# Gardlin/PCR-CG

Measured on AMD Instinct MI355X. Metric: fragment-pairs/s KPFCNN+GCN fwd, 30k-pt pairs, higher is better.
Workload: dtype f32

## Files before the change

include/pcrcg.h:

```cpp
#ifndef PCRCG_H
#define PCRCG_H

#include <stddef.h>
#include <stdint.h>

#ifdef __cplusplus
extern "C" {
#endif

#define PCRCG_OK 0
#define PCRCG_EBADARG (-1)
#define PCRCG_EWORKSPACE (-2)
#define PCRCG_ELAUNCH (-3)
#define PCRCG_ECAPACITY (-4)

#define PCRCG_KPOINTS 15

const char* pcrcg_last_error(void);
#define PCRCG_ABI_VERSION 4
int pcrcg_abi_version(void);

int pcrcg_debug_set(const char* spec);
int pcrcg_debug_release(void);

// ... 1 lines not shown
int pcrcg_grid_subsample_batch(const float* pts, int n, const int* len, int nb, float dl, int max_p,
                               float* out_pts, int* out_len, int* out_m, void* ws, size_t ws_bytes,
                               void* stream);

size_t pcrcg_umap_order_ws_bytes(int m);
int pcrcg_umap_order(const uint64_t* keys, int m, int* order, void* ws, size_t ws_bytes, void* stream);

size_t pcrcg_cellgrid_ws_bytes(int ns, int nb);
int pcrcg_cellgrid_build(const float* sup, int ns, const int* slen, int nb, float radius, void* grid,
                         size_t grid_bytes, void* stream);
int pcrcg_radius_query(const float* q, int nq, const int* qlen, int ns, const int* slen, int nb,
                       float radius, const void* grid, int cols, int64_t* out_idx, int* out_count,
                       int* out_max_count, int* status, void* stream);
int pcrcg_radius_query_ex(const float* q, int nq, const int* qlen, int ns, const int* slen, int nb,
                          float radius, const void* grid, int cols, int64_t* out_idx, int* out_count,
                          int* out_max_count, int* status, int* out_tie_rows, int* out_tie_count, void* stream);
int pcrcg_radius_query_groups(const float* q, int nq, const int* qlen, int ns, const int* slen, int nb, int group,
                              float radius, const void* grid, int cols, int64_t* out_idx, int* out_count,
                              int* out_max_count, int* status, int* out_tie_rows, int* out_tie_count, void* stream);
int pcrcg_radius_query_cells(const void* qgrid, const float* q, int nq, const int* qlen, const void* sgrid, int ns,
                             const int* slen, int nb, int group, float radius, int cols, int64_t* out_idx, int* out_count,
                             int* out_max_count, int* status, int* out_tie_rows, int* out_tie_count, void* stream);
size_t pcrcg_radius_neighbors_ws_bytes(int ns, int nb);
int pcrcg_radius_neighbors_batch(const float* q, int nq, const float* sup, int ns, const int* qlen,
                                 const int* slen, int nb, float radius, int cols, int64_t* out_idx,
                                 int* out_count, int* out_max_count, int* status, void* ws,
                                 size_t ws_bytes, void* stream);

#define PCRCG_MAX_REORDER_JOBS 12
typedef struct pcrcg_reorder_job {
    const float* q;
    const int* qlen;
    const int* rows;
    const int* count;
    int64_t* idx;
    int nq, nbq, cloud0, nrows, max_count, cols;
    float radius;
    int group;
    const float* sup;
    const void* forest;
    int forest_ns, forest_nb;
} pcrcg_reorder_job;
size_t pcrcg_kdforest_ws_bytes(int ns, int nb);
int pcrcg_kdforest_build(const float* sup, int ns, const int* slen, int nb, void* forest, size_t forest_bytes,
                         void* stream);
int pcrcg_radius_reorder(const float* q, int nq, const int* qlen, int nbq, const float* sup, int ns, int nb,
                         const void* forest, int cloud0, float radius, const int* rows, int nrows, const int* count,
                         int max_count, int cols, int64_t* idx, int* status, void* stream);
int pcrcg_radius_reorder_jobs(const pcrcg_reorder_job* jobs, int njobs, const float* sup, int ns, int nb,
                              const void* forest, int* status, void* stream);

size_t pcrcg_kpconv_ws_bytes(int ns);
int pcrcg_kpconv_aggregate(const float* q_pts, int nq, const float* s_pts, int ns, const int64_t* idx,
                           int h, int ld_idx, const float* x, int cin, const float* kp, float extent,
                           float* wf, float* inv_n, void* ws, size_t ws_bytes, void* stream);
int pcrcg_kpconv_aggregate_bf16(const float* q_pts, int nq, const float* s_pts, int ns, const int64_t* idx, int h,
                                int ld_idx, const float* x, int cin, const float* kp, float extent, void* x_bf16,
                                void* wf_bf16, float* inv_n, void* ws, size_t ws_bytes, void* stream);

void pcrcg_profile_kpconv(int enable);
int pcrcg_profile_kpconv_read(float* ms, int* nq, int* h, int* cin, int* cout, int* kind, int cap);

int pcrcg_gemm_f32(const float* a, int lda, const float* b, int ldb, int trans_b, float* c, int ldc, int m,
                   int n, int k, const float* row_scale, const float* bias, void* stream);
size_t pcrcg_gemm_colstats_bytes(int m, int n);
int pcrcg_gemm_f32_colstats(const float* a, int lda, const float* b, int ldb, int trans_b, float* c, int ldc,
                            int m, int n, int k, const float* row_scale, const float* bias, void* colstats,
                            size_t colstats_bytes, int* h_chunks, void* stream);
int pcrcg_gemm_bf16a_f32_colstats(const void* a_bf16, int lda, const float* b, int ldb, float* c, int ldc, int m, int n,
                                  int k, const float* row_scale, const float* bias, void* colstats,
                                  size_t colstats_bytes, int* h_chunks, void* stream);

int pcrcg_gemm_f32_fused(const float* a, int lda, const int64_t* idx, int ld_idx, int ns, const float* zero_row,
                         const void* a_sums, double a_count, float a_eps, float a_slope, const float* b, int ldb,
                         const float* bias, float* c, int ldc, int m, int n, int k, int accumulate, void* stream);

void pcrcg_gemm_set_mode(int mode);
int pcrcg_gemm_get_mode(void);
int pcrcg_gemm_redo_counts(unsigned long long* out2, int reset);
void pcrcg_thread_shares_gpu(int on);

int pcrcg_gather_max(const float* x, int ns, int c, const int64_t* idx, int nq, int h, int ld_idx,
                     float* out, void* stream);
int pcrcg_gather_first(const float* x, int ns, int c, const int64_t* idx, int nq, int ld_idx, float* out,
                       int ld_out, void* stream);
size_t pcrcg_instnorm_ws_bytes(int c);
int pcrcg_instnorm_stats_from_partials(const void* partials, int chunks, int c, double count, float eps,
                                       float* stats, void* stream);
int pcrcg_instnorm_stats(const float* x, int n, int c, int ldx, float eps, float* stats, void* ws,
                         size_t ws_bytes, void* stream);
int pcrcg_instnorm_apply(const float* x, int n, int c, int ldx, const float* stats, const float* res,
                         int ldr, const float* res_stats, float slope, float* y, int ldy, void* stream);
int pcrcg_instnorm_colsums(const float* x, int n, int c, int ldx, void* sums, void* stream);
int pcrcg_instnorm_apply_sums(const float* x, int n, int c, int ldx, const void* sums, double count, float eps,
                              const float* res, int ldr, const void* res_sums, float slope, float* y, int ldy,
                              void* stream);

int pcrcg_fill2d(float* dst, int ld, int rows, int cols, float value, void* stream);
int pcrcg_inject_image_features(const float* fmap, int c, int h, int w, const float* valid, const int64_t* inds2d,
                                const int64_t* inds3d, int n, long row_offset, long n_rows, float* x, int ldx,
                                void* stream);

typedef struct pcrcg_image_frame {
    const float* fmap;
    const float* depth;
    const float* valid;
    float world2camera[16];
    float intrinsics[16];
    float thresh;
    int h, w;
    int depth_h, depth_w;
    int target;
} pcrcg_image_frame;

size_t pcrcg_project_depth_ws_bytes(int n);
int pcrcg_project_depth(const float* points, int n, const float* depth, int h, int w, const float* h_world2camera,
                        const float* h_intrinsics, float thresh, int64_t* inds2d, int64_t* inds3d, int* k, void* ws,
                        size_t ws_bytes, void* stream);
int pcrcg_inject_frames(const float* points, long n_points, long len_src, const pcrcg_image_frame* h_frames, int n_frames,
                        int c, float* x, int ldx, void* stream);
int pcrcg_superglue_valid_maps(const float* keypoints0, int n0, const float* keypoints1, int n1, const int64_t* matches,
                               const float* confidence, int window, int map_w, int map_h, float* src_valid, float* tgt_valid,
                               void* stream);

int pcrcg_knn(const float* coords, int n, int k, int* idx, void* stream);
size_t pcrcg_edgeconv_ws_bytes(int c);
int pcrcg_edgeconv_reduce(const float* ctr, int ld_ctr, const float* nbr, int ld_nbr, const int* idx,
                          int n, int k, int c, float eps, float* emax, int ld_emax, float* stats,
                          void* ws, size_t ws_bytes, void* stream);
int pcrcg_edgeconv_reduce_sums(const float* ctr, int ld_ctr, const float* nbr, int ld_nbr, const int* idx, int n, int k,
                               int c, float* emax, int ld_emax, void* sums, void* stream);
int pcrcg_softmax_rows(float* x, int rows, int cols, int ld, float scale, void* stream);
int pcrcg_attention_supported(int d);
int pcrcg_attention(const float* q, int ldq, const float* k, int ldk, const float* v, int ldv, float* out, int ldo, int n,
                    int ms, int heads, int d, float scale, void* stream);
int pcrcg_softmax_matvec(const float* x, int rows, int cols, int ld, float scale, const float* vec, int ldv, float* y,
                         int ldy, void* stream);

int pcrcg_check_status(const int* status, void* stream);

int pcrcg_copy2d(const float* src, int ld_src, float* dst, int ld_dst, int rows, int cols, void* stream);
int pcrcg_add(const float* a, const float* b, float* dst, long n, void* stream);
int pcrcg_l2norm_rows(const float* src, int ld_src, float* dst, int ld_dst, int rows, int cols, void* stream);
int pcrcg_sigmoid_scores(const float* src, int ld_src, float* dst, int rows, void* stream);

#define PCRCG_MAX_LEVELS 8
#define PCRCG_MAX_BLOCKS 32
#define PCRCG_MAX_GNN 8

enum { PCRCG_BLK_SIMPLE = 0, PCRCG_BLK_RESNETB = 1, PCRCG_BLK_UNARY = 2, PCRCG_BLK_LAST_UNARY = 3,
       PCRCG_BLK_UPSAMPLE = 4 };

typedef struct pcrcg_block {
    int type;
    int layer;
    int strided;
    int in_dim, out_dim;
    int mid_dim;
    float extent;
    const float* kp;
    const float* kp_w;
    const float* kp_wt;
    const float* kp_w_pad;
    int cin_pad;
    const float* unary1;
    const float* unary2;
    const float* shortcut;
    const float* mlp;
    int mlp_ld;
    const float* mlp_skip;
    int mlp_skip_ld, skip_dim;
} pcrcg_block;

typedef struct pcrcg_gnn_layer {
    int cross;
    const float* edge1;
    const float* edge2;
    const float* conv3;
    const float *wq, *bq, *wk, *bk, *wv, *bv;
    const float *wm, *bm;
    const float *w0, *b0;
    const float *w3, *b3;
} pcrcg_gnn_layer;

typedef struct pcrcg_model {
    int n_enc, n_dec, n_gnn;
    pcrcg_block enc[PCRCG_MAX_BLOCKS];
    pcrcg_block dec[PCRCG_MAX_BLOCKS];
    pcrcg_gnn_layer gnn[PCRCG_MAX_GNN];
    int enc_skip[PCRCG_MAX_BLOCKS];
    int dec_concat[PCRCG_MAX_BLOCKS];
    int enc_out_dim, gnn_dim, heads, knn_k, final_dim;
    const float *bottle_w, *bottle_b;
    const float *proj_gnn_w, *proj_gnn_b;
    const float *proj_score_w, *proj_score_b;
    float temperature;
    int feature_bf16;
} pcrcg_model;

typedef struct pcrcg_table { const int64_t* idx; int rows, cols, ld; } pcrcg_table;

typedef struct pcrcg_batch {
    int n_levels;
    const float* points[PCRCG_MAX_LEVELS];
    int n_points[PCRCG_MAX_LEVELS];
    pcrcg_table neighbors[PCRCG_MAX_LEVELS], pools[PCRCG_MAX_LEVELS], upsamples[PCRCG_MAX_LEVELS];
    const float* features;
    int feat_dim;
    int len_src_c;
    const int* stack_lengths[PCRCG_MAX_LEVELS];
} pcrcg_batch;

typedef struct pcrcg_outputs {
    float* feats_f;
    float* scores_overlap;
    float* scores_saliency;
} pcrcg_outputs;

size_t pcrcg_kpfcnn_ws_bytes(const pcrcg_model* model, const pcrcg_batch* batch);
int pcrcg_kpfcnn_forward(const pcrcg_model* model, const pcrcg_batch* batch, const pcrcg_outputs* out, void* ws,
                         size_t ws_bytes, void* stream);

size_t pcrcg_kpfcnn_group_ws_bytes(const pcrcg_model* model, const pcrcg_batch* batches, int n);
int pcrcg_kpfcnn_forward_group(const pcrcg_model* model, const pcrcg_batch* batches, const pcrcg_outputs* outs, int n,
                               void* ws, size_t ws_bytes, void* stream);

typedef struct pcrcg_pyramid_cfg {
    int n_levels;
    float r_conv[PCRCG_MAX_LEVELS], r_pool[PCRCG_MAX_LEVELS], dl[PCRCG_MAX_LEVELS];
    int has_conv[PCRCG_MAX_LEVELS], pooled[PCRCG_MAX_LEVELS], limit[PCRCG_MAX_LEVELS];
    int tie_order;
    int group;
    int up_nearest;
    double shrink;
    void* side_stream;
    void* side_stream2;
} pcrcg_pyramid_cfg;
typedef struct pcrcg_pyramid_restore {
    int njobs;
    pcrcg_reorder_job jobs[PCRCG_MAX_REORDER_JOBS];
    int* tie_status;
} pcrcg_pyramid_restore;
size_t pcrcg_pyramid_ws_bytes(int n0, int nb, const pcrcg_pyramid_cfg* cfg);
int pcrcg_pyramid_build(const float* pts, int n0, const int* len, int nb, const pcrcg_pyramid_cfg* cfg, void* ws,
                        size_t ws_bytes, int* h_scratch, pcrcg_batch* out, int* h_lengths, int* h_status,
                        pcrcg_pyramid_restore* deferred, void* stream);
int pcrcg_pyramid_build_parts(const float* const* pts_parts, const int* n_parts, const int* const* len_parts,
                              const int* nb_parts, int parts, const pcrcg_pyramid_cfg* cfg, void* ws, size_t ws_bytes,
                              int* h_scratch, pcrcg_batch* out, int* h_lengths, int* h_status,
                              pcrcg_pyramid_restore* deferred, void* stream);
int pcrcg_pyramid_restore_run(const pcrcg_pyramid_restore* r, int* h_status, void* stream);

int pcrcg_stream_create(void** stream, int priority);
int pcrcg_stream_destroy(void* stream);
int pcrcg_stream_pipe_classes(void* const* streams, int n, int* cls, void* scratch);

typedef struct pcrcg_ransac_trace {
    int* samples;
    int* pass;
    float* xf32;
    double* xf64;
    int* valid_ids;
    int* counts;
    double* sums;
} pcrcg_ransac_trace;

size_t pcrcg_ransac_ws_bytes(int n, int m, int max_iteration, int max_validation);
int pcrcg_feature_match(const float* src_feat, int ld_src, int n, const float* tgt_feat, int ld_tgt, int m, int c, int mutual,
                        int* corr, int* k, void* ws, size_t ws_bytes, void* stream);
int pcrcg_ransac(const float* src, int n, const float* tgt, int m, const void* grid, const int* corr, int k_max, const int* k,
                 int ransac_n, double threshold, double edge_similarity, int distance_check, int max_iteration,
                 int max_validation, uint64_t seed, double* out_transform, double* out_stats, const pcrcg_ransac_trace* trace,
                 void* ws, size_t ws_bytes, void* stream);

size_t pcrcg_ransac_batch_ws_bytes(int B, int n_total, int m_total, int max_iteration, int max_validation);
int pcrcg_feature_match_batch(const float* src_feat, int ld_src, const int* src_off, int n_total, int n_max,
                              const float* tgt_feat, int ld_tgt, const int* tgt_off, int m_total, int m_max, int c, int B,
                              int* corr, int* k, void* ws, size_t ws_bytes, void* stream);
int pcrcg_ransac_batch(const float* src, const int* src_off, const float* tgt, const int* tgt_off, int m_total, const void* grid,
                       const int* corr, const int* k, int B, int ransac_n, double threshold, double edge_similarity,
                       int distance_check, int max_iteration, int max_validation, const uint64_t* seeds,
                       double* out_transform, double* out_stats, void* ws, size_t ws_bytes, void* stream);

size_t pcrcg_inlier_stats_batch_ws_bytes(int B, int n_total, int m_total);
int pcrcg_inlier_stats_batch(const float* src, const float* src_feat, int ld_src, const int* src_off, int n_total, int n_max,
                             const float* tgt, const float* tgt_feat, int ld_tgt, const int* tgt_off, int m_total, int m_max,
                             int c, int B, const float* rt, const float* thr, int n_thr, int* counts, int* k_mutual,
                             float* dist, int* mutual, int* arg_s, int* arg_t, void* ws, size_t ws_bytes, void* stream);


size_t pcrcg_chamfer_batch_ws_bytes(int B, int n_total, int m_total, int r_total);
int pcrcg_chamfer_batch(const float* src, const int* src_off, int n_total, const float* ref, const int* ref_off, int m_total,
                        const float* raw, const int* raw_off, int r_total, int B, const float* pred, const float* gt,
// ... 15 lines not shown
```

pcrcg_amd/_lib.py:

```python
import ctypes
import os

_HERE = os.path.dirname(os.path.abspath(__file__))
LIB_PATH = os.path.join(_HERE, "libpcrcg_hip.so")


def lib_identity():
    import hashlib
    with open(LIB_PATH, "rb") as f:
        return LIB_PATH, hashlib.sha256(f.read()).hexdigest()[:16]

ABI_VERSION = 4

c_int, c_float, c_void_p, c_size_t = ctypes.c_int, ctypes.c_float, ctypes.c_void_p, ctypes.c_size_t

SIGNATURES = {
    "pcrcg_last_error": (ctypes.c_char_p, []),
    "pcrcg_abi_version": (c_int, []),
    "pcrcg_debug_set": (c_int, [ctypes.c_char_p]),
    "pcrcg_check_status": (c_int, [c_void_p, c_void_p]),
    "pcrcg_grid_subsample_ws_bytes": (c_size_t, [c_int, c_int]),
    "pcrcg_grid_subsample_batch": (c_int, [c_void_p, c_int, c_void_p, c_int, c_float, c_int, c_void_p, c_void_p,
                                           c_void_p, c_void_p, c_size_t, c_void_p]),
    "pcrcg_umap_order_ws_bytes": (c_size_t, [c_int]),
    "pcrcg_umap_order": (c_int, [c_void_p, c_int, c_void_p, c_void_p, c_size_t, c_void_p]),
    "pcrcg_cellgrid_ws_bytes": (c_size_t, [c_int, c_int]),
    "pcrcg_cellgrid_build": (c_int, [c_void_p, c_int, c_void_p, c_int, c_float, c_void_p, c_size_t, c_void_p]),
    "pcrcg_radius_query": (c_int, [c_void_p, c_int, c_void_p, c_int, c_void_p, c_int, c_float, c_void_p, c_int,
                                   c_void_p, c_void_p, c_void_p, c_void_p, c_void_p]),
    "pcrcg_radius_query_ex": (c_int, [c_void_p, c_int, c_void_p, c_int, c_void_p, c_int, c_float, c_void_p, c_int,
                                      c_void_p, c_void_p, c_void_p, c_void_p, c_void_p, c_void_p, c_void_p]),
    "pcrcg_radius_query_groups": (c_int, [c_void_p, c_int, c_void_p, c_int, c_void_p, c_int, c_int, c_float, c_void_p, c_int,
                                          c_void_p, c_void_p, c_void_p, c_void_p, c_void_p, c_void_p, c_void_p]),
    "pcrcg_radius_query_cells": (c_int, [c_void_p, c_void_p, c_int, c_void_p, c_void_p, c_int, c_void_p, c_int, c_int, c_float,
                                         c_int, c_void_p, c_void_p, c_void_p, c_void_p, c_void_p, c_void_p, c_void_p]),
    "pcrcg_kdforest_ws_bytes": (c_size_t, [c_int, c_int]),
    "pcrcg_kdforest_build": (c_int, [c_void_p, c_int, c_void_p, c_int, c_void_p, c_size_t, c_void_p]),
    "pcrcg_radius_reorder": (c_int, [c_void_p, c_int, c_void_p, c_int, c_void_p, c_int, c_int, c_void_p, c_int,
                                     c_float, c_void_p, c_int, c_void_p, c_int, c_int, c_void_p, c_void_p, c_void_p]),
    "pcrcg_radius_reorder_jobs": (c_int, [c_void_p, c_int, c_void_p, c_int, c_int, c_void_p, c_void_p, c_void_p]),
    "pcrcg_radius_neighbors_ws_bytes": (c_size_t, [c_int, c_int]),
    "pcrcg_radius_neighbors_batch": (c_int, [c_void_p, c_int, c_void_p, c_int, c_void_p, c_void_p, c_int, c_float,
                                             c_int, c_void_p, c_void_p, c_void_p, c_void_p, c_void_p, c_size_t,
                                             c_void_p]),
    "pcrcg_kpconv_ws_bytes": (c_size_t, [c_int]),
    "pcrcg_kpconv_aggregate": (c_int, [c_void_p, c_int, c_void_p, c_int, c_void_p, c_int, c_int, c_void_p, c_int,
                                       c_void_p, c_float, c_void_p, c_void_p, c_void_p, c_size_t, c_void_p]),
    "pcrcg_kpconv_aggregate_bf16": (c_int, [c_void_p, c_int, c_void_p, c_int, c_void_p, c_int, c_int, c_void_p, c_int,
                                            c_void_p, c_float, c_void_p, c_void_p, c_void_p, c_void_p, c_size_t,
                                            c_void_p]),
    "pcrcg_profile_kpconv": (None, [c_int]),
    "pcrcg_profile_kpconv_read": (c_int, [c_void_p, c_void_p, c_void_p, c_void_p, c_void_p, c_void_p, c_int]),
    "pcrcg_gemm_f32": (c_int, [c_void_p, c_int, c_void_p, c_int, c_int, c_void_p, c_int, c_int, c_int, c_int,
                               c_void_p, c_void_p, c_void_p]),
    "pcrcg_gemm_colstats_bytes": (c_size_t, [c_int, c_int]),
    "pcrcg_gemm_f32_colstats": (c_int, [c_void_p, c_int, c_void_p, c_int, c_int, c_void_p, c_int, c_int, c_int, c_int,
                                        c_void_p, c_void_p, c_void_p, c_size_t, c_void_p, c_void_p]),
    "pcrcg_gemm_bf16a_f32_colstats": (c_int, [c_void_p, c_int, c_void_p, c_int, c_void_p, c_int, c_int, c_int, c_int,
                                              c_void_p, c_void_p, c_void_p, c_size_t, c_void_p, c_void_p]),
    "pcrcg_gemm_f32_fused": (c_int, [c_void_p, c_int, c_void_p, c_int, c_int, c_void_p, c_void_p, ctypes.c_double, c_float,
                                     c_float, c_void_p, c_int, c_void_p, c_void_p, c_int, c_int, c_int, c_int, c_int, c_void_p]),
    "pcrcg_gemm_set_mode": (None, [c_int]),
    "pcrcg_gemm_get_mode": (c_int, []),
    "pcrcg_gemm_redo_counts": (c_int, [c_void_p, c_int]),
    "pcrcg_instnorm_stats_from_partials": (c_int, [c_void_p, c_int, c_int, ctypes.c_double, c_float, c_void_p,
                                                   c_void_p]),
    "pcrcg_gather_max": (c_int, [c_void_p, c_int, c_int, c_void_p, c_int, c_int, c_int, c_void_p, c_void_p]),
    "pcrcg_gather_first": (c_int, [c_void_p, c_int, c_int, c_void_p, c_int, c_int, c_void_p, c_int, c_void_p]),
    "pcrcg_instnorm_ws_bytes": (c_size_t, [c_int]),
    "pcrcg_instnorm_stats": (c_int, [c_void_p, c_int, c_int, c_int, c_float, c_void_p, c_void_p, c_size_t, c_void_p]),
    "pcrcg_instnorm_apply": (c_int, [c_void_p, c_int, c_int, c_int, c_void_p, c_void_p, c_int, c_void_p, c_float,
                                     c_void_p, c_int, c_void_p]),
    "pcrcg_instnorm_colsums": (c_int, [c_void_p, c_int, c_int, c_int, c_void_p, c_void_p]),
    "pcrcg_instnorm_apply_sums": (c_int, [c_void_p, c_int, c_int, c_int, c_void_p, ctypes.c_double, c_float, c_void_p, c_int,
                                          c_void_p, c_float, c_void_p, c_int, c_void_p]),
    "pcrcg_fill2d": (c_int, [c_void_p, c_int, c_int, c_int, c_float, c_void_p]),
    "pcrcg_inject_image_features": (c_int, [c_void_p, c_int, c_int, c_int, c_void_p, c_void_p, c_void_p, c_int, ctypes.c_long,
                                            ctypes.c_long, c_void_p, c_int, c_void_p]),
    "pcrcg_project_depth_ws_bytes": (c_size_t, [c_int]),
    "pcrcg_project_depth": (c_int, [c_void_p, c_int, c_void_p, c_int, c_int, c_void_p, c_void_p, c_float, c_void_p, c_void_p,
                                    c_void_p, c_void_p, c_size_t, c_void_p]),
    "pcrcg_inject_frames": (c_int, [c_void_p, ctypes.c_long, ctypes.c_long, c_void_p, c_int, c_int, c_void_p, c_int, c_void_p]),
    "pcrcg_superglue_valid_maps": (c_int, [c_void_p, c_int, c_void_p, c_int, c_void_p, c_void_p, c_int, c_int, c_int, c_void_p,
                                           c_void_p, c_void_p]),
    "pcrcg_knn": (c_int, [c_void_p, c_int, c_int, c_void_p, c_void_p]),
    "pcrcg_edgeconv_ws_bytes": (c_size_t, [c_int]),
    "pcrcg_edgeconv_reduce": (c_int, [c_void_p, c_int, c_void_p, c_int, c_void_p, c_int, c_int, c_int, c_float,
                                      c_void_p, c_int, c_void_p, c_void_p, c_size_t, c_void_p]),
    "pcrcg_edgeconv_reduce_sums": (c_int, [c_void_p, c_int, c_void_p, c_int, c_void_p, c_int, c_int, c_int, c_void_p, c_int,
                                           c_void_p, c_void_p]),
    "pcrcg_softmax_rows": (c_int, [c_void_p, c_int, c_int, c_int, c_float, c_void_p]),
    "pcrcg_attention_supported": (c_int, [c_int]),
    "pcrcg_attention": (c_int, [c_void_p, c_int, c_void_p, c_int, c_void_p, c_int, c_void_p, c_int, c_int, c_int, c_int,
                                c_int, c_float, c_void_p]),
    "pcrcg_softmax_matvec": (c_int, [c_void_p, c_int, c_int, c_int, c_float, c_void_p, c_int, c_void_p, c_int, c_void_p]),
    "pcrcg_copy2d": (c_int, [c_void_p, c_int, c_void_p, c_int, c_int, c_int, c_void_p]),
    "pcrcg_add": (c_int, [c_void_p, c_void_p, c_void_p, ctypes.c_long, c_void_p]),
    "pcrcg_l2norm_rows": (c_int, [c_void_p, c_int, c_void_p, c_int, c_int, c_int, c_void_p]),
    "pcrcg_sigmoid_scores": (c_int, [c_void_p, c_int, c_void_p, c_int, c_void_p]),
    "pcrcg_kpfcnn_ws_bytes": (c_size_t, [c_void_p, c_void_p]),
    "pcrcg_kpfcnn_group_ws_bytes": (c_size_t, [c_void_p, c_void_p, c_int]),
    "pcrcg_kpfcnn_forward_group": (c_int, [c_void_p, c_void_p, c_void_p, c_int, c_void_p, c_size_t, c_void_p]),
    "pcrcg_kpfcnn_forward": (c_int, [c_void_p, c_void_p, c_void_p, c_void_p, c_size_t, c_void_p]),
    "pcrcg_pyramid_ws_bytes": (c_size_t, [c_int, c_int, c_void_p]),
    "pcrcg_pyramid_build": (c_int, [c_void_p, c_int, c_void_p, c_int, c_void_p, c_void_p, c_size_t, c_void_p, c_void_p,
                                    c_void_p, c_void_p, c_void_p, c_void_p]),
    "pcrcg_pyramid_build_parts": (c_int, [c_void_p, c_void_p, c_void_p, c_void_p, c_int, c_void_p, c_void_p, c_size_t, c_void_p,
                                          c_void_p, c_void_p, c_void_p, c_void_p, c_void_p]),
    "pcrcg_pyramid_restore_run": (c_int, [c_void_p, c_void_p, c_void_p]),
    "pcrcg_debug_release": (c_int, []),
    "pcrcg_stream_pipe_classes": (c_int, [c_void_p, c_int, c_void_p, c_void_p]),
    "pcrcg_thread_shares_gpu": (None, [c_int]),
    "pcrcg_stream_create": (c_int, [c_void_p, c_int]),
    "pcrcg_stream_destroy": (c_int, [c_void_p]),
    "pcrcg_ransac_ws_bytes": (c_size_t, [c_int, c_int, c_int, c_int]),
    "pcrcg_feature_match": (c_int, [c_void_p, c_int, c_int, c_void_p, c_int, c_int, c_int, c_int, c_void_p, c_void_p,
                                    c_void_p, c_size_t, c_void_p]),
    "pcrcg_ransac": (c_int, [c_void_p, c_int, c_void_p, c_int, c_void_p, c_void_p, c_int, c_void_p, c_int, ctypes.c_double,
                             ctypes.c_double, c_int, c_int, c_int, ctypes.c_uint64, c_void_p, c_void_p, c_void_p, c_void_p,
                             c_size_t, c_void_p]),
    "pcrcg_ransac_batch_ws_bytes": (c_size_t, [c_int, c_int, c_int, c_int, c_int]),
    "pcrcg_feature_match_batch": (c_int, [c_void_p, c_int, c_void_p, c_int, c_int, c_void_p, c_int, c_void_p, c_int, c_int,
                                          c_int, c_int, c_void_p, c_void_p, c_void_p, c_size_t, c_void_p]),
    "pcrcg_ransac_batch": (c_int, [c_void_p, c_void_p, c_void_p, c_void_p, c_int, c_void_p, c_void_p, c_void_p, c_int, c_int,
                                   ctypes.c_double, ctypes.c_double, c_int, c_int, c_int, c_void_p, c_void_p, c_void_p,
                                   c_void_p, c_size_t, c_void_p]),
    "pcrcg_inlier_stats_batch_ws_bytes": (c_size_t, [c_int, c_int, c_int]),
    "pcrcg_inlier_stats_batch": (c_int, [c_void_p, c_void_p, c_int, c_void_p, c_int, c_int, c_void_p, c_void_p, c_int, c_void_p,
                                         c_int, c_int, c_int, c_int, c_void_p, c_void_p, c_int, c_void_p, c_void_p, c_void_p,
                                         c_void_p, c_void_p, c_void_p, c_void_p, c_size_t, c_void_p]),
    "pcrcg_chamfer_batch_ws_bytes": (c_size_t, [c_int, c_int, c_int, c_int]),
    "pcrcg_chamfer_batch": (c_int, [c_void_p, c_void_p, c_int, c_void_p, c_void_p, c_int, c_void_p, c_void_p, c_int, c_int,
                                    c_void_p, c_void_p, c_void_p, c_void_p, c_void_p, c_void_p, c_void_p, c_void_p, c_void_p,
                                    c_void_p, c_size_t, c_void_p]),
    "pcrcg_res50unet_arena_bytes": (c_size_t, [c_int]),
    "pcrcg_res50unet_pack": (c_int, [c_void_p, c_int, c_int, c_void_p, c_void_p]),
    "pcrcg_res50unet_ws_bytes": (c_size_t, [c_int, c_int, c_int]),
    "pcrcg_res50unet_forward": (c_int, [c_void_p, c_void_p, c_int, c_int, c_void_p, c_int, c_int, c_int, c_int, c_int,
                                        c_void_p, c_void_p, c_size_t, c_void_p]),
    "pcrcg_gemm_f32_ex": (c_int, [c_void_p, c_int, c_int, c_void_p, c_int, c_int, c_void_p, c_int, c_int, c_int, c_int,
                                  c_void_p, c_void_p, c_void_p]),
    "pcrcg_gemm_f32_grad": (c_int, [c_void_p, c_int, c_int, c_void_p, c_int, c_int, c_void_p, c_int, c_int, c_int, c_int,
                                  c_void_p, c_void_p, c_int, c_void_p]),
    "pcrcg_kpconv_backward_dx": (c_int, [c_void_p, c_int, c_void_p, c_int, c_void_p, c_int, c_int, c_void_p, c_int,
                                         c_void_p, c_float, c_void_p, c_void_p]),
    "pcrcg_kpconv_forward_ws_bytes": (c_size_t, [c_int, c_int, c_int]),
    "pcrcg_kpconv_forward": (c_int, [c_void_p, c_int, c_void_p, c_int, c_void_p, c_int, c_int, c_void_p, c_int, c_void_p,
                                     c_float, c_void_p, c_int, c_void_p, c_int, c_void_p, c_size_t, c_void_p]),
    "pcrcg_kpconv_backward_ws_bytes": (c_size_t, [c_int, c_int, c_int]),
    "pcrcg_kpconv_backward": (c_int, [c_void_p, c_int, c_void_p, c_int, c_void_p, c_int, c_int, c_int, c_void_p, c_float,
# ... 68 lines not shown
```

pcrcg_amd/csrc/common.h:

```cpp
#pragma once
#include <hip/hip_runtime.h>

#include <cstdarg>
#include <cstdint>
#include <cstdio>
#include <mutex>

#include "pcrcg.h"

namespace pcrcg {

void set_error(const char* fmt, ...);

inline hipStream_t as_stream(void* s) { return reinterpret_cast<hipStream_t>(s); }

struct Carver {
    char* base;
    size_t cap;
    size_t off = 0;
    Carver(void* ws, size_t bytes) : base(static_cast<char*>(ws)), cap(bytes) {}
    template <typename T>
    T* take(size_t count) {
        size_t bytes = (count * sizeof(T) + 255) & ~size_t(255);
        T* p = reinterpret_cast<T*>(base + off);
// ... 5 lines not shown
inline size_t carve_bytes(size_t count, size_t elem) { return (count * elem + 255) & ~size_t(255); }

size_t scan_ws_bytes(int n);
int exclusive_scan_i32(const int* in, int* out, int n, int* total, void* ws, hipStream_t stream);

constexpr int kWave = 64;

int grid_subsample_bound(const float* pts, int n_bound, const int* len, int nb, float dl, int max_p, float* out_pts,
                         int* out_len, int* out_m, int out_cap, int* overflow, void* ws, size_t ws_bytes, hipStream_t stream);

bool instnorm_pack_ok(int c, int ldx, int ldy);
int instnorm_apply_pack(const float* x, int n, int c, int ldx, const float* stats, const double* sums, double count, float eps,
                        float slope, float* y, int ldy, const float* s_pts, float4* pk, hipStream_t st);
float4* kpconv_pk_ptr(void* ws, size_t ws_bytes, int ns);

void gemm_x6_release_det();
void trainops_release_det();
void conv2d_release_det();

int kdforest_build_levels(const float* sup, int ns, const int* slen, int nb, int per_level, const int* level_base, void* forest,
                          size_t forest_bytes, hipStream_t stream);

int radius_fast_cap();
int radius_query_pass(const float* q, int nq, const int* qlen, int ns, const int* slen, int nb, int group, float radius,
                      const void* grid, int cols, int64_t* out_idx, int* out_count, int* out_max_count, int* status,
                      int* out_tie_rows, int* out_tie_count, hipStream_t st, int pass);

bool gemm_x6_shared();
void gemm_x6_set_shared(int on);
int radius_cells_pass(const void* qgrid, const float* q, int nq, const int* qlen, const void* sgrid, int ns, const int* slen,
                      int nb, int group, float radius, int cols, int64_t* out_idx, int* out_count, int* out_max_count,
                      int* status, int* out_tie_rows, int* out_tie_count, hipStream_t st, int pass);
constexpr int kRadiusRedoStatus = 4;

struct GemmExtra {
    const long long* a_idx = nullptr;
    int a_idx_ld = 0, a_ns = 0;
    const float* a_zero = nullptr;
    bool accumulate = false;
    const double* a_sums = nullptr;
    double a_count = 0.0;
    float a_eps = 1e-5f, a_slope = 1.0f;
    int grad_operand = 0;
};

struct GemmPair {
    const float* a = nullptr;
    float* c = nullptr;
    int m = 0;
    const float* row_scale = nullptr;
    void* colstats = nullptr;
    int* h_chunks = nullptr;
    bool c_zeroed = false;
    const long long* a_idx = nullptr;
    int a_ns = 0;
    const double* a_sums = nullptr;
    double a_count = 0.0;
};
struct GemmGroup {
    int n = 0;
    GemmPair p[3];
};

int kpconv_pack(const float* x, int ns, int cin, const float* s_pts, void* ws, size_t ws_bytes, hipStream_t st,
                unsigned short* x_bf16 = nullptr);
int kpconv_aggregate_rows(const float* q_pts, int nq, const float* s_pts, int ns, const int64_t* idx, int h, int ld_idx,
                          const float* x, int cin, const float* kp, float extent, float* wf, float* inv_n, void* ws,
                          size_t ws_bytes, hipStream_t st, bool pack, bool stream_out, int c1_ld = 0);
int kpconv_aggregate_bf16(const float* q_pts, int nq, const float* s_pts, int ns, const int64_t* idx, int h, int ld_idx,
                          const float* x, unsigned short* x_bf16, int cin, const float* kp, float extent,
                          unsigned short* wf_bf16, float* inv_n, void* ws, size_t ws_bytes, hipStream_t st);

struct NormJob {
    const float* x; const double* sums; const float* res; const double* res_sums; float* y;
    const float* s_pts; float4* pk;
    int n; double count;
    float* stats_out = nullptr;
};
int instnorm_apply_sums_multi(const NormJob* jobs, int count, int c, int ldx, float eps, int ldr, float slope, int ldy, bool pack,
                              hipStream_t st);

struct GatherJob { const float* x; const int64_t* idx; float* out; int ns, nq, h, ld_idx; };
int gather_max_multi(const GatherJob* jobs, int count, int c, hipStream_t st);
int heads_multi(const float* const* x, const int* rows, int count, int ld, int fd, float* const* feats, float* const* s_ov,
                float* const* s_sal, hipStream_t st);
int copy2d_multi(const float* const* src, float* const* dst, const int* rows, int count, int ld_src, int ld_dst, int cols,
                 hipStream_t st);
int instnorm_colsums_multi(const float* const* x, double* const* sums, const int* n, int count, int c, int ldx, hipStream_t st);

struct EdgeCloud {
    const float* ctr; const float* nbr; const int* idx; float* emax; double* sums; int n, k;
};
bool edgeconv_rows_ok(const EdgeCloud* cl, int count, int ld_ctr, int ld_nbr, int ld_emax, int c);
int edgeconv_rows_multi(const EdgeCloud* cl, int count, int ld_ctr, int ld_nbr, int ld_emax, int c, bool atomic, int* nchunks_out,
                        hipStream_t st);

struct AttnCloud { const float* q; const float* k; const float* v; float* out; int n, ms; };
bool attention_mfma_ok(const AttnCloud* cl, int count, int ldq, int ldk, int ldv, int d);
int attention_mfma_multi(const AttnCloud* cl, int count, int ldq, int ldk, int ldv, int ldo, int heads, int d, float scale,
                         hipStream_t st);
bool attention_bwd_mfma_ok(int n, int ms, int d, int ldq, int ldk, int ldv, int ld_do);
int attention_bwd_mfma(const float* q, int ldq, const float* k, int ldk, const float* v, int ldv, const float* o, int ldo,
                       const float* d_o, int ld_do, float* dq, int ld_dq, float* dk, int ld_dk, float* dv, int ld_dv, int n, int ms,
                       int heads, int d, float scale, hipStream_t st);

struct DebugOpts {
    int stat_sums = 1;
    int stat_sums_rows = 1 << 30;
    int att_mfma = 1;
    int radius_blocks = 0;
    int kd_blocks = 0;
    int att_tq = 16;
    int kd_spin_limit = 0;
    int gemm_log = 0;
    int x6_tile = -1, x6_splitk = 0, x6_t1 = 1, x6_t2 = 1, x6_order = -1, x6_big = 0, x6_h2 = 1;
    int train_side_stream = 1;
    int gemm_tile = -1, gemm_splitk = 0, gemm_split_target = 768;
    int deterministic = 0;
    int bwd_mfma = 1;
};
const DebugOpts& debug_opts();

struct KpProfScope {
    hipStream_t st;
    hipEvent_t a, b;
    int nq, h, cin, cout, kind;
    bool on;
    KpProfScope(hipStream_t s, int nq, int h, int cin, int cout, int kind);
    ~KpProfScope();
};

}

#define PCRCG_CHECK_ARG(cond)                                                        \
    do {                                                                             \
        if (!(cond)) {                                                               \
            pcrcg::set_error("%s: bad argument: %s", __func__, #cond);               \
            return PCRCG_EBADARG;                                                    \
        }                                                                            \
    } while (0)

#define PCRCG_CHECK_WS(carver)                                                                     \
    do {                                                                                           \
        if (!(carver).ok()) {                                                                      \
            pcrcg::set_error("%s: workspace too small (%zu needed, %zu given)", __func__,          \
                             (carver).off, (carver).cap);                                          \
            return PCRCG_EWORKSPACE;                                                               \
        }                                                                                          \
    } while (0)

#define PCRCG_CHECK_HIP(expr)                                                                  \
    do {                                                                                       \
        hipError_t e_ = (expr);                                                                \
        if (e_ != hipSuccess) {                                                                \
            pcrcg::set_error("%s: %s failed: %s", __func__, #expr, hipGetErrorString(e_));     \
            return PCRCG_ELAUNCH;                                                              \
        }                                                                                      \
    } while (0)

#define PCRCG_CHECK_LAUNCH() PCRCG_CHECK_HIP(hipGetLastError())

namespace pcrcg {
inline hipError_t grant_max_dyn_lds(const void* kern) {
    hipFuncAttributes at;
    hipError_t e = hipFuncGetAttributes(&at, kern);
    if (e != hipSuccess) return e;
// ... 18 lines not shown
```

pcrcg_amd/csrc/pointops.hip:

```cpp
#include "common.h"

namespace pcrcg {
namespace {

constexpr int kWavesPerBlock = 4;

struct GatherMulti { const float* x[4]; const long long* idx[4]; float* out[4]; int ns[4], nq[4], h[4], ld_idx[4]; };
template <bool VEC4>
__global__ void __launch_bounds__(kWavesPerBlock * 64) k_gather_max(GatherMulti mm, int c, int nchunk) {
    const int g = blockIdx.y;
    const float* __restrict__ x = mm.x[g];
    const long long* __restrict__ idx = mm.idx[g];
    float* __restrict__ out = mm.out[g];
    const int ns = mm.ns[g], nq = mm.nq[g], h = mm.h[g], ld_idx = mm.ld_idx[g];
    const int lane = threadIdx.x & 63;
    const long item = (long)blockIdx.x * kWavesPerBlock + __builtin_amdgcn_readfirstlane((int)(threadIdx.x >> 6));
    if (item >= (long)nq * nchunk) return;
    const int q = (int)(item / nchunk), chunk = (int)(item - (long)q * nchunk);
    const long long* row = idx + (long)q * ld_idx;
    if (VEC4) {
        const int cb = chunk * 64 + lane;
        if (cb >= (c >> 2)) return;
        float4 m = make_float4(0.f, 0.f, 0.f, 0.f);
        bool any = false;
#pragma unroll 4
        for (int j = 0; j < h; ++j) {
            const long long i = row[j];
            float4 v = make_float4(0.f, 0.f, 0.f, 0.f);
            if (i >= 0 && i < ns) v = reinterpret_cast<const float4*>(x + i * c)[cb];
            if (!any) { m = v; any = true; }
            else { m.x = fmaxf(m.x, v.x); m.y = fmaxf(m.y, v.y); m.z = fmaxf(m.z, v.z); m.w = fmaxf(m.w, v.w); }
        }
        reinterpret_cast<float4*>(out + (long)q * c)[cb] = m;
    } else {
        const int cc = chunk * 64 + lane;
        if (cc >= c) return;
        float m = 0.f;
        bool any = false;
#pragma unroll 4
        for (int j = 0; j < h; ++j) {
            const long long i = row[j];
            const float v = (i >= 0 && i < ns) ? x[i * c + cc] : 0.f;
            m = any ? fmaxf(m, v) : v;
            any = true;
        }
        out[(long)q * c + cc] = m;
    }
}

__global__ void __launch_bounds__(256) k_gather_first(const float* __restrict__ x, int ns, int c,
                                                       const long long* __restrict__ idx, int nq, int ld_idx,
                                                       float* __restrict__ out, int ld_out) {
    const int lane = threadIdx.x & 63;
    const int q = blockIdx.x * 4 + __builtin_amdgcn_readfirstlane((int)(threadIdx.x >> 6));
    if (q >= nq) return;
    const long long i = idx[(long)q * ld_idx];
    const bool real = i >= 0 && i < ns;
    for (int cc = lane; cc < c; cc += 64) out[(long)q * ld_out + cc] = real ? x[i * c + cc] : 0.f;
}

constexpr int kStatChunks = 128;

struct ColsMulti { const float* x[4]; double* partial[4]; int n[4]; };
template <bool ATOMIC>
__global__ void __launch_bounds__(256) k_colstats_partial(ColsMulti mm, int c, int ldx) {
    const float* __restrict__ x = mm.x[blockIdx.z];
    double* __restrict__ partial = mm.partial[blockIdx.z];
    const int n = mm.n[blockIdx.z];
    __shared__ double s_sum[4][64], s_sq[4][64];
    const int lane = threadIdx.x & 63, rl = threadIdx.x >> 6;
    const int ch = blockIdx.y * 64 + lane;
    const int chunk = blockIdx.x, nchunks = gridDim.x;
    const long rows_per = ((long)n + nchunks - 1) / nchunks;
    const long r0 = chunk * rows_per, r1 = min((long)n, r0 + rows_per);
    double s = 0.0, sq = 0.0;
    if (ch < c) {
        long r = r0 + rl;
        for (; r + 12 < r1; r += 16) {
            const float v0 = x[r * ldx + ch], v1 = x[(r + 4) * ldx + ch], v2 = x[(r + 8) * ldx + ch],
                        v3 = x[(r + 12) * ldx + ch];
            s += ((double)v0 + (double)v1) + ((double)v2 + (double)v3);
            sq += ((double)v0 * v0 + (double)v1 * v1) + ((double)v2 * v2 + (double)v3 * v3);
        }
        for (; r < r1; r += 4) {
            const double v = (double)x[r * ldx + ch];
            s += v;
            sq += v * v;
        }
    }
    s_sum[rl][lane] = s;
    s_sq[rl][lane] = sq;
    __syncthreads();
    if (rl == 0 && ch < c) {
        s = (s_sum[0][lane] + s_sum[1][lane]) + (s_sum[2][lane] + s_sum[3][lane]);
        sq = (s_sq[0][lane] + s_sq[1][lane]) + (s_sq[2][lane] + s_sq[3][lane]);
        if (ATOMIC) {
            if (r0 < r1) {
                unsafeAtomicAdd(&partial[ch], s);
                unsafeAtomicAdd(&partial[(long)c + ch], sq);
            }
        } else {
            partial[(long)ch * nchunks + chunk] = s;
            partial[((long)c + ch) * nchunks + chunk] = sq;
        }
    }
}

__global__ void __launch_bounds__(256) k_colstats_final(const double* __restrict__ partial, int nchunks, int c,
                                                         double count, float eps, float* __restrict__ stats) {
    const int lane = threadIdx.x & 63;
    const int ch = blockIdx.x * (blockDim.x >> 6) + (threadIdx.x >> 6);
    if (ch >= c) return;
    double s = 0.0, sq = 0.0;
    for (int k = lane; k < nchunks; k += 64) {
        s += partial[(long)ch * nchunks + k];
        sq += partial[((long)c + ch) * nchunks + k];
    }
#pragma unroll
    for (int d = 32; d >= 1; d >>= 1) {
        s += __shfl_xor(s, d, 64);
        sq += __shfl_xor(sq, d, 64);
    }
    if (lane != 0) return;
    const double mean = s / count;
    double var = sq / count - mean * mean;
    if (var < 0.0) var = 0.0;
    stats[2 * ch] = (float)mean;
    stats[2 * ch + 1] = (float)(1.0 / sqrt(var + (double)eps));
}
// ... 187 lines not shown
    const int c4 = c / 4;
    if (stats) {
        const long total = (long)n * c4;
        hipLaunchKernelGGL(k_instnorm_apply4_pack, dim3((unsigned)((total + 255) / 256)), dim3(256), 0, st, x, n, c4, ldx, stats,
                           slope, y, ldy, s_pts, pk);
    } else {
        NormJob one{x, sums, nullptr, nullptr, y, s_pts, pk, n, count};
        return instnorm_apply_sums_multi(&one, 1, c, ldx, eps, 0, slope, ldy, true, st);
    }
    PCRCG_CHECK_LAUNCH();
    return PCRCG_OK;
}

int instnorm_apply_sums_multi(const NormJob* jobs, int count, int c, int ldx, float eps, int ldr, float slope, int ldy, bool pack,
                              hipStream_t st) {
    PCRCG_CHECK_ARG(jobs && count >= 1 && count <= 4 && c >= 4 && c % 4 == 0);
    const int c4 = c / 4;
    NormMulti mm;
    int nmax = 0;
    for (int g = 0; g < 4; ++g) {
        const NormJob& j = jobs[g < count ? g : 0];
        mm.x[g] = j.x; mm.sums[g] = j.sums; mm.res[g] = j.res; mm.res_sums[g] = j.res_sums; mm.y[g] = j.y;
        mm.s_pts[g] = j.s_pts; mm.pk[g] = j.pk; mm.n[g] = g < count ? j.n : 0; mm.count[g] = j.count;
        mm.stats_out[g] = g < count ? j.stats_out : nullptr;
        if (g < count) {
            PCRCG_CHECK_ARG(j.n >= 0 && j.x && j.sums && j.y && j.count >= 1.0);
            PCRCG_CHECK_ARG((j.res != nullptr) == (jobs[0].res != nullptr) && (j.res_sums != nullptr) == (jobs[0].res_sums != nullptr));
            nmax = j.n > nmax ? j.n : nmax;
        }
    }
    if (nmax == 0) return PCRCG_OK;
    const int rp = 256 / (c4 < 256 ? c4 : 256);
    int rows_per_block = rp * 8;
    while (rows_per_block > rp && (long)(nmax + rows_per_block - 1) / rows_per_block * count < 256) rows_per_block -= rp;
    const dim3 grid((unsigned)((nmax + rows_per_block - 1) / rows_per_block), count);
    if (pack)
        hipLaunchKernelGGL(k_instnorm_apply4_sums_pack, grid, dim3(256), 0, st, mm, c4, ldx, eps, slope, ldy, rows_per_block);
    else if (!jobs[0].res)
        hipLaunchKernelGGL(k_instnorm_apply4_sums<0>, grid, dim3(256), 0, st, mm, c4, ldx, eps, ldr, slope, ldy, rows_per_block);
    else if (!jobs[0].res_sums)
        hipLaunchKernelGGL(k_instnorm_apply4_sums<1>, grid, dim3(256), 0, st, mm, c4, ldx, eps, ldr, slope, ldy, rows_per_block);
    else
        hipLaunchKernelGGL(k_instnorm_apply4_sums<2>, grid, dim3(256), 0, st, mm, c4, ldx, eps, ldr, slope, ldy, rows_per_block);
    PCRCG_CHECK_LAUNCH();
    return PCRCG_OK;
}

size_t colstats_ws_bytes(int c) { return carve_bytes((size_t)kStatChunks * 2 * (size_t)(c > 0 ? c : 1), sizeof(double)); }

int colstats_finalize(const double* partial, int nchunks, int c, double count, float eps, float* stats,
                      hipStream_t st) {
    hipLaunchKernelGGL(k_colstats_final, dim3((c + 3) / 4), dim3(256), 0, st, partial, nchunks, c, count, eps, stats);
    PCRCG_CHECK_LAUNCH();
    return PCRCG_OK;
}
int colstats_chunks() { return kStatChunks; }

int gather_max_multi(const GatherJob* jobs, int count, int c, hipStream_t st) {
    PCRCG_CHECK_ARG(jobs && count >= 1 && count <= 4 && c >= 1);
    GatherMulti mm;
    bool vec = c % 4 == 0;
    int nq_max = 0;
    for (int g = 0; g < 4; ++g) {
        const GatherJob& j = jobs[g < count ? g : 0];
        mm.x[g] = j.x; mm.idx[g] = reinterpret_cast<const long long*>(j.idx); mm.out[g] = j.out;
        mm.ns[g] = j.ns; mm.nq[g] = g < count ? j.nq : 0; mm.h[g] = j.h; mm.ld_idx[g] = j.ld_idx;
        if (g < count) {
            PCRCG_CHECK_ARG(j.ns >= 0 && j.nq >= 0 && j.h >= 1 && j.ld_idx >= j.h && (j.nq == 0 || (j.x && j.idx && j.out)));
            vec = vec && ((reinterpret_cast<uintptr_t>(j.x) | reinterpret_cast<uintptr_t>(j.out)) & 15) == 0;
            nq_max = j.nq > nq_max ? j.nq : nq_max;
        }
    }
    if (nq_max == 0) return PCRCG_OK;
    const int per_wave = vec ? 256 : 64;
    const int nchunk = (c + per_wave - 1) / per_wave;
    const long items = (long)nq_max * nchunk;
    const dim3 grid((unsigned)((items + kWavesPerBlock - 1) / kWavesPerBlock), count);
    if (vec) hipLaunchKernelGGL(k_gather_max<true>, grid, dim3(kWavesPerBlock * 64), 0, st, mm, c, nchunk);
    else hipLaunchKernelGGL(k_gather_max<false>, grid, dim3(kWavesPerBlock * 64), 0, st, mm, c, nchunk);
    PCRCG_CHECK_LAUNCH();
    return PCRCG_OK;
}

int instnorm_colsums_multi(const float* const* x, double* const* sums, const int* n, int count, int c, int ldx, hipStream_t st) {
    PCRCG_CHECK_ARG(count >= 1 && count <= 4 && c >= 1 && ldx >= c);
    ColsMulti mm;
    int nmax = 0;
    for (int g = 0; g < 4; ++g) {
        const int k = g < count ? g : 0;
        PCRCG_CHECK_ARG(n[k] >= 1 && x[k] && sums[k]);
        mm.x[g] = x[k]; mm.partial[g] = sums[k]; mm.n[g] = n[k];
        if (g < count) nmax = n[k] > nmax ? n[k] : nmax;
    }
    int chunks = (nmax + 63) / 64;
    if (chunks > kStatChunks) chunks = kStatChunks;
    if (debug_opts().deterministic) chunks = 1;
    hipLaunchKernelGGL(k_colstats_partial<true>, dim3(chunks, (c + 63) / 64, count), dim3(256), 0, st, mm, c, ldx);
    PCRCG_CHECK_LAUNCH();
    return PCRCG_OK;
}

}

using namespace pcrcg;

extern "C" {

int pcrcg_gather_max(const float* x, int ns, int c, const int64_t* idx, int nq, int h, int ld_idx,
                     float* out, void* stream) {
    PCRCG_CHECK_ARG(ns >= 0 && c >= 1 && nq >= 0 && h >= 1 && ld_idx >= h);
    if (nq == 0) return PCRCG_OK;
    PCRCG_CHECK_ARG(x && idx && out);
    const GatherJob one{x, idx, out, ns, nq, h, ld_idx};
    return gather_max_multi(&one, 1, c, as_stream(stream));
}

int pcrcg_gather_first(const float* x, int ns, int c, const int64_t* idx, int nq, int ld_idx, float* out,
                       int ld_out, void* stream) {
    PCRCG_CHECK_ARG(ns >= 0 && c >= 1 && nq >= 0 && ld_idx >= 1 && ld_out >= c);
    if (nq == 0) return PCRCG_OK;
    PCRCG_CHECK_ARG(x && idx && out);
    hipLaunchKernelGGL(k_gather_first, dim3((nq + 3) / 4), dim3(256), 0, as_stream(stream), x, ns, c,
                       reinterpret_cast<const long long*>(idx), nq, ld_idx, out, ld_out);
    PCRCG_CHECK_LAUNCH();
    return PCRCG_OK;
}

size_t pcrcg_instnorm_ws_bytes(int c) { return colstats_ws_bytes(c); }

int pcrcg_instnorm_stats_from_partials(const void* partials, int chunks, int c, double count, float eps,
                                       float* stats, void* stream) {
    PCRCG_CHECK_ARG(partials && stats && chunks >= 1 && c >= 1 && count >= 1.0);
    return colstats_finalize(static_cast<const double*>(partials), chunks, c, count, eps, stats, as_stream(stream));
}

int pcrcg_instnorm_stats(const float* x, int n, int c, int ldx, float eps, float* stats, void* ws,
                         size_t ws_bytes, void* stream) {
    PCRCG_CHECK_ARG(n >= 1 && c >= 1 && ldx >= c && x && stats && ws);
    Carver cv(ws, ws_bytes);
    double* partial = cv.take<double>((size_t)kStatChunks * 2 * c);
    PCRCG_CHECK_WS(cv);
    hipStream_t st = as_stream(stream);
    {
        ColsMulti mm;
        for (int g = 0; g < 4; ++g) { mm.x[g] = x; mm.partial[g] = partial; mm.n[g] = n; }
        hipLaunchKernelGGL(k_colstats_partial<false>, dim3(kStatChunks, (c + 63) / 64, 1), dim3(256), 0, st, mm, c, ldx);
    }
    return colstats_finalize(partial, kStatChunks, c, (double)n, eps, stats, st);
}

int pcrcg_instnorm_colsums(const float* x, int n, int c, int ldx, void* sums, void* stream) {
    PCRCG_CHECK_ARG(n >= 1 && c >= 1 && ldx >= c && x && sums);
    const float* xs[1] = {x};
    double* ss[1] = {static_cast<double*>(sums)};
    return instnorm_colsums_multi(xs, ss, &n, 1, c, ldx, as_stream(stream));
}

int pcrcg_instnorm_apply_sums(const float* x, int n, int c, int ldx, const void* sums, double count, float eps,
                              const float* res, int ldr, const void* res_sums, float slope, float* y, int ldy,
                              void* stream) {
    PCRCG_CHECK_ARG(n >= 0 && c >= 4 && c % 4 == 0 && ldx >= c && ldy >= c && count >= 1.0);
    if (n == 0) return PCRCG_OK;
    PCRCG_CHECK_ARG(x && sums && y && (!res || ldr >= c) && (!res_sums || res));
    const int c4 = c / 4;
    auto al16 = [](const void* p) { return (reinterpret_cast<uintptr_t>(p) & 15) == 0; };
    PCRCG_CHECK_ARG((c4 <= 256 ? 256 % c4 == 0 : c4 % 256 == 0) && ldx % 4 == 0 && ldy % 4 == 0 && al16(x) && al16(y) &&
                    (!res || (ldr % 4 == 0 && al16(res))));
    NormJob one{x, static_cast<const double*>(sums), res, static_cast<const double*>(res_sums), y, nullptr, nullptr, n, count};
    return instnorm_apply_sums_multi(&one, 1, c, ldx, eps, ldr, slope, ldy, false, as_stream(stream));
}

int pcrcg_instnorm_apply(const float* x, int n, int c, int ldx, const float* stats, const float* res,
                         int ldr, const float* res_stats, float slope, float* y, int ldy, void* stream) {
    PCRCG_CHECK_ARG(n >= 0 && c >= 1 && ldx >= c && ldy >= c);
    if (n == 0) return PCRCG_OK;
    PCRCG_CHECK_ARG(x && stats && y);
    PCRCG_CHECK_ARG(!res || ldr >= c);
    auto al16 = [](const void* p) { return (reinterpret_cast<uintptr_t>(p) & 15) == 0; };
    const bool vec = c % 4 == 0 && ldx % 4 == 0 && ldy % 4 == 0 && al16(x) && al16(y) && al16(stats) &&
                     (!res || (ldr % 4 == 0 && al16(res))) && (!res_stats || al16(res_stats));
    if (vec) {
        const long total = (long)n * (c / 4);
        hipLaunchKernelGGL(k_instnorm_apply4, dim3((unsigned)((total + 255) / 256)), dim3(256), 0, as_stream(stream), x,
                           n, c / 4, ldx, stats, res, ldr, res_stats, slope, y, ldy);
    } else {
        const long total = (long)n * c;
        hipLaunchKernelGGL(k_instnorm_apply, dim3((unsigned)((total + 255) / 256)), dim3(256), 0, as_stream(stream), x,
                           n, c, ldx, stats, res, ldr, res_stats, slope, y, ldy);
    }
    PCRCG_CHECK_LAUNCH();
    return PCRCG_OK;
}
}
```

pcrcg_amd/csrc/pyramid.hip:

```cpp
#include <time.h>

#include <cmath>
#include <cstdlib>
#include <vector>

#include "common.h"

namespace pcrcg {
namespace {

inline double now_us() {
    timespec ts;
    clock_gettime(CLOCK_MONOTONIC, &ts);
    return ts.tv_sec * 1e6 + ts.tv_nsec * 1e-3;
}

__global__ void k_probe_many(int* sink, int spin) {
    int x = threadIdx.x;
    for (int i = 0; i < spin; ++i) x = x * 1664525 + 1013904223;
    if (x == 0x7fffffff) sink[0] = x;
}
__global__ void k_probe_tiny(int* sink) {
    if (threadIdx.x == 1234567) sink[1] = 1;
}
// ... 128 lines not shown
    int* metas = A.take<int>(meta_ints);
    int* m_dev = metas + MS * max_tables;
    int* overflow = m_dev + L;
    int* tie_status = overflow + 1;
    if (!A.ok()) return PCRCG_EWORKSPACE;

    std::vector<TableRec> tables;
    tables.reserve(max_tables);
    if (!dry) {
        PCRCG_CHECK_HIP(hipMemsetAsync(metas, 0, sizeof(int) * meta_ints, st));
        size_t row = 0, cloud = 0;
        for (int i = 0; i < in.count; ++i) {
            if (in.n[i] > 0)
                PCRCG_CHECK_HIP(hipMemcpyAsync(level_pts[0] + 3 * row, in.pts[i], sizeof(float) * 3 * (size_t)in.n[i], hipMemcpyDeviceToDevice, st));
            PCRCG_CHECK_HIP(hipMemcpyAsync(lens_all + cloud, in.len[i], sizeof(int) * in.nb[i], hipMemcpyDeviceToDevice, st));
            row += (size_t)in.n[i];
            cloud += (size_t)in.nb[i];
        }
        PCRCG_CHECK_HIP(hipMemsetD32Async(reinterpret_cast<hipDeviceptr_t>(feats), 0x3f800000, (size_t)(n0 > 0 ? n0 : 1), st));
    }

    hipStream_t sub_st = cfg->side_stream ? as_stream(cfg->side_stream) : st;
    hipStream_t f_st = cfg->side_stream2 ? as_stream(cfg->side_stream2) : sub_st;
    EventBox events;
    auto order = [&](hipStream_t a, hipStream_t b) -> int {
        if (a == b || dry) return PCRCG_OK;
        hipEvent_t ev;
        PCRCG_PROPAGATE(events.make(&ev));
        PCRCG_CHECK_HIP(hipEventRecord(ev, a));
        PCRCG_CHECK_HIP(hipStreamWaitEvent(b, ev, 0));
        return PCRCG_OK;
    };
    const bool one_forest = !want_ties || f_st == st || L < 2;
    void* forest[2] = {nullptr, nullptr};
    size_t forest_b[2] = {0, 0};
    int forest_ns[2] = {0, 0}, forest_nb[2] = {0, 0};
    int level_base[PCRCG_MAX_LEVELS] = {};
    auto build_forest = [&](int which) -> int {
        if (!want_ties || (which == 1 && L < 2)) return PCRCG_OK;
        const int first = which == 1 ? 1 : 0, last = which == 0 ? 0 : L - 1, slot = which == 1 ? 1 : 0;
        for (int l = first; l <= last; ++l) level_base[l - first] = (int)((level_pts[l] - level_pts[first]) / 3);
        forest_ns[slot] = level_base[last - first] + cap[last];
        forest_nb[slot] = (last - first + 1) * nb;
        forest_b[slot] = pcrcg_kdforest_ws_bytes(forest_ns[slot], forest_nb[slot]);
        forest[slot] = A.raw(forest_b[slot]);
        if (!A.ok()) return PCRCG_EWORKSPACE;
        if (dry) return PCRCG_OK;
        PCRCG_PROPAGATE(order(which == 0 ? st : sub_st, f_st));
        return kdforest_build_levels(level_pts[first], forest_ns[slot], lens_all + (size_t)first * nb, forest_nb[slot],
                                     last > first ? nb : 0, level_base, forest[slot], forest_b[slot], f_st);
    };

    auto add_table = [&](int kind, int level, int q_level, const void* grid, const void* qgrid, float radius, const float* q,
                         const int* qlen, int nq, int ns, const int* slen, int limit, int sup_level) -> int {
        TableRec t;
        t.kind = kind; t.level = level; t.q_level = q_level;
        t.idx = A.take<int64_t>((size_t)nq * limit);
        t.counts = want_ties ? A.take<int>((size_t)nq) : nullptr;
        t.ties = want_ties ? A.take<int>((size_t)nq) : nullptr;
        t.meta = metas + MS * tables.size();
        t.q = q; t.qlen = qlen; t.nq = nq; t.limit = limit; t.sup_level = sup_level; t.radius = radius;
        t.grid = grid; t.ns = ns; t.slen = slen; t.qgrid = qgrid;
        if (!A.ok()) return PCRCG_EWORKSPACE;
        if (!dry)
            PCRCG_PROPAGATE(radius_cells_pass(t.qgrid, q, nq, qlen, grid, ns, slen, nb, group, radius, limit, t.idx, t.counts,
                                              t.meta, t.meta + P, t.ties, want_ties ? t.meta + P + 1 : nullptr, st, 1));
        tables.push_back(t);
        return PCRCG_OK;
    };
    auto build_grid = [&](const float* sup, int ns, const int* slen, float radius, void** grid) -> int {
        const size_t gb = pcrcg_cellgrid_ws_bytes(ns, nb);
        *grid = A.raw(gb);
        if (!A.ok()) return PCRCG_EWORKSPACE;
        if (!dry) PCRCG_PROPAGATE(pcrcg_cellgrid_build(sup, ns, slen, nb, radius, *grid, gb, st));
        return PCRCG_OK;
    };

    const size_t sub_wsb = L > 1 ? pcrcg_grid_subsample_ws_bytes(cap[0], nb) : 0;
    void* sub_ws = L > 1 ? A.raw(sub_wsb) : nullptr;
    if (!A.ok()) return PCRCG_EWORKSPACE;

    void* carried = nullptr;
    float carried_r = 0.f;
    PCRCG_PROPAGATE(order(st, sub_st));
    if (!one_forest) PCRCG_PROPAGATE(build_forest(0));
    else if (L == 1) PCRCG_PROPAGATE(build_forest(0));
    for (int l = 0; l < L; ++l) {
        const int limit = cfg->limit[l];
        const float r_conv = cfg->r_conv[l], r_pool = cfg->r_pool[l];
        float* pts = level_pts[l];
        int* lens = lens_all + (size_t)l * nb;
        const int n = cap[l];
        void* grid = nullptr;
        float grid_r = 0.f;
        const bool pooled = cfg->pooled[l] && l + 1 < L;
        if (!pooled && l + 1 < L) {
            set_error("pcrcg_pyramid_build: level %d of %d is not pooled", l, L);
            return PCRCG_EBADARG;
        }
        if (pooled && !dry)
            PCRCG_PROPAGATE(grid_subsample_bound(pts, n, lens, nb, cfg->dl[l], 0, level_pts[l + 1], lens + nb, m_dev + l, cap[l + 1],
                                                 overflow, sub_ws, sub_wsb, sub_st));
        if (pooled && l + 2 == L) PCRCG_PROPAGATE(build_forest(one_forest ? 2 : 1));
        if (cfg->has_conv[l]) {
            if (carried && carried_r == r_conv) { grid = carried; grid_r = carried_r; }
            else { PCRCG_PROPAGATE(build_grid(pts, n, lens, r_conv, &grid)); grid_r = r_conv; }
            PCRCG_PROPAGATE(add_table(0, l, l, grid, grid, r_conv, pts, lens, n, n, lens, limit, l));
        }
        carried = nullptr;
        if (pooled) {
            float* sub = level_pts[l + 1];
            int* sub_len = lens + nb;
            const int m = cap[l + 1];
            if (grid == nullptr || grid_r != r_pool) {
                PCRCG_PROPAGATE(build_grid(pts, n, lens, r_pool, &grid));
                grid_r = r_pool;
            }
            PCRCG_PROPAGATE(order(sub_st, st));
            void* up_grid = nullptr;
            PCRCG_PROPAGATE(build_grid(sub, m, sub_len, 2 * r_pool, &up_grid));
            PCRCG_PROPAGATE(add_table(1, l, l + 1, grid, up_grid, r_pool, sub, sub_len, m, n, lens, limit, l));
            PCRCG_PROPAGATE(add_table(2, l, l, up_grid, grid, 2 * r_pool, pts, lens, n, m, sub_len, cfg->up_nearest ? 1 : limit, l + 1));
            carried = up_grid;
            carried_r = 2 * r_pool;
        }
    }
    if (dry) return PCRCG_OK;
    hipEvent_t forests_done = nullptr;
    if (want_ties && f_st != st) {
        PCRCG_PROPAGATE(events.make(&forests_done));
        PCRCG_CHECK_HIP(hipEventRecord(forests_done, f_st));
    }

    const int nt = (int)tables.size();
    const int meta_words = MS * max_tables + L + 1;
    PCRCG_PROPAGATE(fetch(h_scratch, metas, meta_words, lens_all, L * nb, st, enqueue));
    if (forests_done) PCRCG_CHECK_HIP(hipStreamWaitEvent(st, forests_done, 0));
    const int* hm = h_scratch + 1;
    if (hm[MS * max_tables + L] != 0) {
        set_error("pcrcg_pyramid_build: a level keeps more rows than pcrcg_pyramid_cfg::shrink = %.3f allows -- call again with a "
                  "larger bound (1.0 always fits)", cfg->shrink);
        return PCRCG_EWORKSPACE;
    }
    for (int i = 0; i < L * nb; ++i) h_lengths[i] = hm[meta_words + i];
    int level_n[PCRCG_MAX_LEVELS];
    for (int l = 0; l < L; ++l) {
        level_n[l] = 0;
        for (int c = 0; c < nb; ++c) level_n[l] += h_lengths[(size_t)l * nb + c];
    }
    {
        int redone = 0;
        for (int i = 0; i < nt; ++i) {
            int widest = 0;
            for (int p = 0; p < P; ++p) widest = hm[MS * i + p] > widest ? hm[MS * i + p] : widest;
            const bool handed_over = (hm[MS * i + P] & kRadiusRedoStatus) != 0;
            if (widest <= radius_fast_cap() && !handed_over) continue;
            const TableRec& t = tables[i];
            PCRCG_PROPAGATE(radius_query_pass(t.q, t.nq, t.qlen, t.ns, t.slen, nb, group, t.radius, t.grid, t.limit, t.idx,
                                              t.counts, t.meta, t.meta + P, t.ties, want_ties ? t.meta + P + 1 : nullptr, st,
                                              2));
            ++redone;
        }
        if (redone) PCRCG_PROPAGATE(fetch(h_scratch, metas, meta_words, lens_all, L * nb, st));
    }
    auto group_rows = [&](int l, int p, int* row0, int* rows) {
        const int c0 = group > 0 ? p * group : 0, c1 = group > 0 ? c0 + group : nb;
        int a = 0, r = 0;
        for (int c = 0; c < c1; ++c) (c < c0 ? a : r) += h_lengths[(size_t)l * nb + c];
        *row0 = a;
        *rows = r;
    };
    for (int p = 0; p < P; ++p) {
        pcrcg_batch& o = out[p];
        o.n_levels = L;
        int row0, rows;
        group_rows(0, p, &row0, &rows);
        o.features = feats + row0;
        o.feat_dim = 1;
        o.len_src_c = h_lengths[(size_t)(L - 1) * nb + (group > 0 ? p * group : 0)];
        for (int l = 0; l < L; ++l) {
            group_rows(l, p, &row0, &rows);
            o.points[l] = level_pts[l] + 3 * (size_t)row0;
            o.n_points[l] = rows;
            o.stack_lengths[l] = lens_all + (size_t)l * nb + (group > 0 ? p * group : 0);
            o.neighbors[l] = pcrcg_table{nullptr, rows, 0, 1};
            o.pools[l] = pcrcg_table{nullptr, 0, 0, 1};
            o.upsamples[l] = pcrcg_table{nullptr, 0, 0, 1};
        }
    }
    pcrcg_pyramid_restore local;
    pcrcg_pyramid_restore& R = deferred ? *deferred : local;
    R.njobs = 0;
    for (int i = 0; i < nt; ++i) {
        TableRec& t = tables[i];
        const int status = hm[MS * i + P], tie_rows = hm[MS * i + P + 1];
        if (status != 0) {
            set_error("pcrcg_pyramid_build: radius search capacity exceeded (table %d)", i);
            return PCRCG_ECAPACITY;
        }
        int widest = 0;
        for (int p = 0; p < P; ++p) {
            const int max_count = hm[MS * i + p];
            widest = max_count > widest ? max_count : widest;
            const int cols = max_count < t.limit ? (max_count > 0 ? max_count : 0) : t.limit;
            int row0, rows;
            group_rows(t.q_level, p, &row0, &rows);
            pcrcg_table tab{t.idx + (size_t)row0 * t.limit, rows, cols, t.limit};
            if (t.kind == 0) out[p].neighbors[t.level] = tab;
            else if (t.kind == 1) out[p].pools[t.level] = tab;
            else out[p].upsamples[t.level] = tab;
        }
        if (want_ties && widest > 0 && tie_rows > 0 && R.njobs < PCRCG_MAX_REORDER_JOBS) {
            pcrcg_reorder_job& j = R.jobs[R.njobs++];
            const int fi = (one_forest || t.sup_level == 0) ? 0 : 1;
            j.q = t.q; j.qlen = t.qlen; j.rows = t.ties; j.count = t.counts; j.idx = t.idx;
            j.nq = level_n[t.q_level]; j.nbq = nb; j.cloud0 = one_forest ? t.sup_level * nb : (fi == 0 ? 0 : (t.sup_level - 1) * nb);
            j.nrows = tie_rows;
            j.max_count = widest < 8192 ? widest : 8192;
            j.cols = t.limit; j.radius = t.radius; j.group = group;
            j.sup = level_pts[fi]; j.forest = forest[fi]; j.forest_ns = forest_ns[fi]; j.forest_nb = forest_nb[fi];
        }
    }
    R.tie_status = tie_status;
    if (!deferred) return pcrcg_pyramid_restore_run(&R, h_status, st);
    return PCRCG_OK;
}

extern "C" {

size_t pcrcg_pyramid_ws_bytes(int n0, int nb, const pcrcg_pyramid_cfg* cfg) {
    if (!cfg || n0 < 0 || nb < 1 || cfg->n_levels < 1 || cfg->n_levels > PCRCG_MAX_LEVELS) return 0;
    Arena A(nullptr, 0, true);
    const Parts none{nullptr, nullptr, nullptr, nullptr, 0};
    if (pyramid_run(none, n0, nb, cfg, A, nullptr, nullptr, nullptr, nullptr, nullptr, nullptr) != PCRCG_OK) return 0;
    return A.peak + 4096;
}

int pcrcg_stream_create(void** stream, int priority) {
    PCRCG_CHECK_ARG(stream != nullptr);
    hipStream_t st = nullptr;
    PCRCG_CHECK_HIP(hipStreamCreateWithPriority(&st, hipStreamNonBlocking, priority));
    *stream = st;
    return PCRCG_OK;
}

int pcrcg_stream_pipe_classes(void* const* streams, int n, int* cls, void* scratch) {
    PCRCG_CHECK_ARG(streams && cls && scratch && n >= 1 && n <= 64);
    int* sink = static_cast<int*>(scratch);
    PCRCG_CHECK_HIP(hipDeviceSynchronize());
    for (int i = 0; i < n; ++i) hipLaunchKernelGGL(k_probe_tiny, dim3(1), dim3(64), 0, as_stream(streams[i]), sink);
    PCRCG_CHECK_HIP(hipDeviceSynchronize());
    const int blocks = 2000000;
    double t0 = now_us();
    hipLaunchKernelGGL(k_probe_many, dim3(blocks), dim3(64), 0, as_stream(streams[0]), sink, 64);
    PCRCG_CHECK_HIP(hipStreamSynchronize(as_stream(streams[0])));
    const double big_us = now_us() - t0;
    if (big_us < 400.0) {
        set_error("pcrcg_stream_pipe_classes: the dispatch-bound probe kernel took only %.0f us", big_us);
        return PCRCG_ELAUNCH;
    }
    int reps[8], nrep = 0;
    auto shares = [&](int a, int b, bool* out) -> int {
        int yes = 0, no = 0;
        for (int trial = 0; trial < 10 && yes < 2 && no < 2; ++trial) {
            const double launch = now_us();
            hipLaunchKernelGGL(k_probe_many, dim3(blocks), dim3(64), 0, as_stream(streams[a]), sink, 64);
            const double start = now_us();
            while (now_us() - start < 150.0) {}
            const double a0 = now_us();
            hipLaunchKernelGGL(k_probe_tiny, dim3(1), dim3(64), 0, as_stream(streams[b]), sink);
            const double a1 = now_us();
// ... 86 lines not shown
```

pcrcg_amd/csrc/radius.hip:

```cpp
#include <hip/hip_ext.h>

#include "block_scan.h"
#include <cstdlib>

#include "common.h"
#include "cellgrid.h"

namespace pcrcg {
namespace {

constexpr int kListCapFast = 256;
constexpr int kListCapFull = 1024;
constexpr long long kRedoMark = -2;
constexpr int kQueryWaves = 4;
constexpr int kTieCap = 256;

constexpr int kRedoStatus = 4;
constexpr int kCellCand = 1024;
constexpr int kCellListCap = 128;
constexpr unsigned kPadKey = 0x7FFFFFFFu;
constexpr int kCellTieCap = 512;
constexpr int kCellMaxCells = 256;
constexpr int kCellQ = 64;

// ... 790 lines not shown
                          int* out_max_count, int* status, int* out_tie_rows, int* out_tie_count, void* stream) {
    return pcrcg_radius_query_groups(q, nq, qlen, ns, slen, nb, 0, radius, grid, cols, out_idx, out_count, out_max_count,
                                     status, out_tie_rows, out_tie_count, stream);
}

int pcrcg_radius_query_groups(const float* q, int nq, const int* qlen, int ns, const int* slen, int nb, int group,
                              float radius, const void* grid, int cols, int64_t* out_idx, int* out_count,
                              int* out_max_count, int* status, int* out_tie_rows, int* out_tie_count, void* stream) {
    return pcrcg::radius_query_pass(q, nq, qlen, ns, slen, nb, group, radius, grid, cols, out_idx, out_count, out_max_count,
                                    status, out_tie_rows, out_tie_count, as_stream(stream), 0);
}
}

namespace pcrcg {
int radius_fast_cap() { return kListCapFast; }

int radius_query_pass(const float* q, int nq, const int* qlen, int ns, const int* slen, int nb, int group, float radius,
                      const void* grid, int cols, int64_t* out_idx, int* out_count, int* out_max_count, int* status,
                      int* out_tie_rows, int* out_tie_count, hipStream_t st, int pass) {
    PCRCG_CHECK_ARG(nq >= 0 && ns >= 0 && nb >= 1 && cols >= 1 && group >= 0);
    PCRCG_CHECK_ARG((out_tie_rows == nullptr) == (out_tie_count == nullptr));
    PCRCG_CHECK_ARG(qlen && slen && grid && out_idx && out_max_count);
    PCRCG_CHECK_ARG(nq == 0 || q);
    (void)slen;
    if (nq == 0) return PCRCG_OK;
    bool ok;
    GridView g = grid_view(const_cast<void*>(grid), grid_bytes(ns, nb), ns, nb, &ok);
    const float r2 = radius * radius;
    int blocks = (nq + kQueryWaves - 1) / kQueryWaves;
    const int max_blocks_env = debug_opts().radius_blocks;
    const int max_blocks = max_blocks_env > 0 ? max_blocks_env : 256 * 2;
    if (blocks > max_blocks) blocks = max_blocks;
    if (pass != 2) {
        KpProfScope ev(st, nq, cols, ns, 0, 4);
        hipExtLaunchKernelGGL((k_radius_query<kListCapFast, false, kQueryWaves>), dim3(blocks), dim3(kQueryWaves * 64), 0, st, ev.a,
                              ev.b, 0, q, nq, qlen, nb, r2, g, cols, reinterpret_cast<long long*>(out_idx), out_count,
                              out_max_count, status, out_tie_rows, out_tie_count, group);
    }
    const int redo_blocks = blocks < 64 ? blocks : 64;
    if (pass != 1)
        hipLaunchKernelGGL((k_radius_query<kListCapFull, true, 1>), dim3(redo_blocks), dim3(64), 0, st, q, nq, qlen, nb, r2, g,
                           cols, reinterpret_cast<long long*>(out_idx), out_count, out_max_count, status, out_tie_rows,
                           out_tie_count, group);
    PCRCG_CHECK_LAUNCH();
    return PCRCG_OK;
}
}

namespace pcrcg {
int radius_cells_pass(const void* qgrid, const float* q, int nq, const int* qlen, const void* sgrid, int ns, const int* slen,
                      int nb, int group, float radius, int cols, int64_t* out_idx, int* out_count, int* out_max_count,
                      int* status, int* out_tie_rows, int* out_tie_count, hipStream_t st, int pass) {
    PCRCG_CHECK_ARG(nq >= 0 && ns >= 0 && nb >= 1 && cols >= 1 && group >= 0 && radius > 0.0f);
    PCRCG_CHECK_ARG((out_tie_rows == nullptr) == (out_tie_count == nullptr));
    PCRCG_CHECK_ARG(qgrid && sgrid && out_idx && out_max_count);
    PCRCG_CHECK_ARG(pass == 1 || (q && qlen && slen));
    if (nq == 0) return PCRCG_OK;
    bool ok;
    GridView gq = grid_view(const_cast<void*>(qgrid), grid_bytes(nq, nb), nq, nb, &ok);
    GridView gs = grid_view(const_cast<void*>(sgrid), grid_bytes(ns, nb), ns, nb, &ok);
    const float r2 = radius * radius;
    const double reach = (double)radius * (1.0 + 1e-6);
    const int max_blocks_env = debug_opts().radius_blocks;
    const int max_blocks = max_blocks_env > 0 ? max_blocks_env : (pass == 1 ? 512 : 1536);
    int blocks = (nq + 7) / 8;
    if (blocks > max_blocks) blocks = max_blocks;
    CellArgs ca;
    ca.qhdr = gq.hdr; ca.qtick = gq.qtick; ca.qspts = gq.spts; ca.ckey = gq.ckey; ca.cinfo = gq.cinfo;
    ca.shdr = gs.hdr; ca.soff = gs.soff; ca.tab = gs.tab; ca.spts = gs.spts;
    ca.out_idx = reinterpret_cast<long long*>(out_idx); ca.out_count = out_count; ca.out_max = out_max_count;
    ca.status = status; ca.tie_rows = out_tie_rows; ca.tie_count = out_tie_count;
    ca.reach = reach; ca.r2 = r2; ca.nb = nb; ca.cols = cols; ca.group = group;
    if (pass != 1) PCRCG_CHECK_HIP(hipMemsetAsync(gq.qtick, 0, 16 * kTickStride * sizeof(int), st));
    {
        KpProfScope ev(st, nq, cols, ns, 1, 4);
        hipExtLaunchKernelGGL((k_radius_cells<kCellCand, kCellListCap, kQueryWaves>), dim3(blocks), dim3(kQueryWaves * 64), 0, st,
                              ev.a, ev.b, 0, ca);
    }
    PCRCG_CHECK_LAUNCH();
    if (pass == 1) return PCRCG_OK;
    return radius_query_pass(q, nq, qlen, ns, slen, nb, group, radius, sgrid, cols, out_idx, out_count, out_max_count, status,
                             out_tie_rows, out_tie_count, st, 2);
}
}

extern "C" {

int pcrcg_radius_query_cells(const void* qgrid, const float* q, int nq, const int* qlen, const void* sgrid, int ns,
                             const int* slen, int nb, int group, float radius, int cols, int64_t* out_idx, int* out_count,
                             int* out_max_count, int* status, int* out_tie_rows, int* out_tie_count, void* stream) {
    return pcrcg::radius_cells_pass(qgrid, q, nq, qlen, sgrid, ns, slen, nb, group, radius, cols, out_idx, out_count,
                                    out_max_count, status, out_tie_rows, out_tie_count, as_stream(stream), 0);
}

size_t pcrcg_radius_neighbors_ws_bytes(int ns, int nb) { return pcrcg_cellgrid_ws_bytes(ns, nb); }

int pcrcg_radius_neighbors_batch(const float* q, int nq, const float* sup, int ns, const int* qlen,
                                 const int* slen, int nb, float radius, int cols, int64_t* out_idx,
                                 int* out_count, int* out_max_count, int* status, void* ws,
                                 size_t ws_bytes, void* stream) {
    PCRCG_CHECK_ARG(out_max_count != nullptr);
    hipLaunchKernelGGL(k_zero2, dim3(1), dim3(1), 0, as_stream(stream), out_max_count, status);
    PCRCG_PROPAGATE(pcrcg_cellgrid_build(sup, ns, slen, nb, radius, ws, ws_bytes, stream));
    return pcrcg_radius_query(q, nq, qlen, ns, slen, nb, radius, ws, cols, out_idx, out_count, out_max_count,
                              status, stream);
}
}
```

pcrcg_amd/csrc/runner.hip:

```cpp
#include <vector>

#include <cstdlib>

#include "common.h"

namespace pcrcg {
bool gemm_bt_accumulates(int m, int n, int k, long m_total = 0);
int gemm_bt_colstats(const float* a, int lda, const float* b, int ldb, float* c, int ldc, int m, int n, int k,
                     const float* row_scale, const float* bias, void* colstats, size_t colstats_bytes, int* h_chunks,
                     hipStream_t st, bool c_zeroed, bool colstats_sums = false);
int gemm_bf16a_bt_colstats(const void* a_bf16, int lda, const float* b, int ldb, float* c, int ldc, int m, int n, int k,
                           const float* row_scale, const float* bias, void* colstats, size_t colstats_bytes,
                           int* h_chunks, hipStream_t st, bool c_zeroed, bool colstats_sums);
bool gemm_colstats_sums_ok();
bool gemm_extra_ok();
int gemm_bt_extra(const float* a, int lda, const float* b, int ldb, float* c, int ldc, int m, int n, int k, hipStream_t st,
                  bool c_zeroed, const GemmExtra& ex, const float* bias = nullptr, void* colstats = nullptr,
                  size_t colstats_bytes = 0, int* h_chunks = nullptr, bool colstats_sums = false);
bool gemm_pair_ok();
int gemm_bt_colstats_pair(const float* a, int lda, const float* b, int ldb, float* c, int ldc, int m, int n, int k,
                          const float* row_scale, const float* bias, void* colstats, size_t colstats_bytes, int* h_chunks,
                          hipStream_t st, bool c_zeroed, bool colstats_sums, const GemmGroup* grp);
int gemm_bt_extra_pair(const float* a, int lda, const float* b, int ldb, float* c, int ldc, int m, int n, int k, hipStream_t st,
                       bool c_zeroed, const GemmExtra& ex, const float* bias, void* colstats, size_t colstats_bytes,
// ... 387 lines not shown
    norm_act(c, t, 0.1f, y, &ts);
    c.release(m);
    return y;
}

bool norm_act_pack(Ctx& c, const Batches& B, int layer, const Mat& t, float slope, const Mat& u, Stat* ts, void* const* kp_ws,
                   const size_t* kp_ws_bytes) {
    if (c.bf16 || !instnorm_pack_ok(t.cols, t.ld, u.ld) || u.ld != u.cols) return false;
    const size_t m = c.mark();
    float* stats = static_cast<float*>(c.raw(sizeof(float) * 2 * t.cols));
    const size_t wsb = pcrcg_instnorm_ws_bytes(t.cols);
    void* ws = c.raw(wsb);
    fill_sums(c, t, ts);
    if (c.live() && all_sums(c, ts) && c.G <= 4) {
        NormJob jobs[GMAX];
        bool ok = true;
        for (int g = 0; g < c.G; ++g) {
            float4* pk = kpconv_pk_ptr(kp_ws[g], kp_ws_bytes[g], t.rows[g]);
            ok = ok && pk != nullptr && ((reinterpret_cast<uintptr_t>(t.p[g]) | reinterpret_cast<uintptr_t>(u.p[g])) & 15) == 0;
            jobs[g] = NormJob{t.p[g], static_cast<const double*>(ts->partials[g]), nullptr, nullptr, u.p[g], B.b[g]->points[layer], pk,
                              t.rows[g], (double)(t.rows[g] > 0 ? t.rows[g] : 1)};
        }
        if (ok) {
            c.check(instnorm_apply_sums_multi(jobs, c.G, t.cols, t.ld, 1e-5f, 0, slope, u.ld, true, c.st));
            c.release(m);
            return true;
        }
    }
    if (c.live())
        for (int g = 0; g < c.G; ++g) {
            const float* s_pts = B.b[g]->points[layer];
            float4* pk = kpconv_pk_ptr(kp_ws[g], kp_ws_bytes[g], t.rows[g]);
            if (!pk) c.check(PCRCG_EWORKSPACE);
            else if (ts && ts->chunks[g] == -1)
                c.check(instnorm_apply_pack(t.p[g], t.rows[g], t.cols, t.ld, nullptr, static_cast<const double*>(ts->partials[g]),
                                            (double)t.rows[g], 1e-5f, slope, u.p[g], u.ld, s_pts, pk, c.st));
            else {
                col_stats(c, t, g, ts, stats, ws, wsb);
                c.check(instnorm_apply_pack(t.p[g], t.rows[g], t.cols, t.ld, stats, nullptr, 0.0, 1e-5f, slope, u.p[g], u.ld, s_pts,
                                            pk, c.st));
            }
        }
    c.release(m);
    return true;
}

Mat resnet_block(Ctx& c, const Batches& B, const pcrcg_block& blk, const Mat& feats) {
    int nq[GMAX];
    out_rows(c, B, blk, nq);
    Mat y = c.mat(nq, blk.out_dim);
    const size_t m = c.mark();
    Mat x = feats;
    void* kp_ws[GMAX] = {};
    size_t kp_wsb[GMAX] = {};
    bool packed = false;
    if (blk.unary1) {
        Mat t = c.gemm_out(feats.rows, blk.mid_dim, feats.cols), u = c.mat(feats.rows, blk.mid_dim);
        Stat ts = stat_buffer(c, t.rows, t.cols);
        linear(c, feats, blk.unary1, feats.cols, nullptr, t, &ts);
        if (blk.mid_dim % 4 == 0 && !(blk.kp_w_pad && blk.cin_pad > blk.mid_dim)) {
            for (int g = 0; g < c.G; ++g) {
                kp_wsb[g] = pcrcg_kpconv_ws_bytes(feats.rows[g]);
                kp_ws[g] = c.raw(kp_wsb[g]);
            }
            packed = norm_act_pack(c, B, blk.layer, t, 0.1f, u, &ts, kp_ws, kp_wsb);
        }
        if (!packed) norm_act(c, t, 0.1f, u, &ts);
        x = u;
    }
    Mat k = c.gemm_out(nq, blk.mid_dim, PCRCG_KPOINTS * kp_cin(blk, x)), kn = c.mat(nq, blk.mid_dim);
    Stat ks = stat_buffer(c, nq, blk.mid_dim);
    kpconv(c, B, blk, x, k, &ks, packed ? kp_ws : nullptr);
    Mat u2 = c.gemm_out(nq, blk.out_dim, blk.mid_dim);
    Stat u2s = stat_buffer(c, nq, blk.out_dim);
    if (!linear_norm(c, k, &ks, 0.1f, blk.unary2, blk.mid_dim, nullptr, u2, &u2s)) {
        norm_act(c, k, 0.1f, kn, &ks);
        linear(c, kn, blk.unary2, blk.mid_dim, nullptr, u2, &u2s);
    }
    Mat sc = feats;
    if (blk.strided) {
        sc = c.mat(nq, feats.cols);
        if (c.live() && c.G <= 4) {
            GatherJob jobs[GMAX];
            for (int g = 0; g < c.G; ++g) {
                const pcrcg_table& t = B.b[g]->pools[blk.layer];
                jobs[g] = GatherJob{feats.p[g], t.idx, sc.p[g], feats.rows[g], nq[g], t.cols, t.ld};
            }
            c.check(gather_max_multi(jobs, c.G, feats.cols, c.st));
        } else if (c.live())
            for (int g = 0; g < c.G; ++g) {
                const pcrcg_table& t = B.b[g]->pools[blk.layer];
                c.check(pcrcg_gather_max(feats.p[g], feats.rows[g], feats.cols, t.idx, nq[g], t.cols, t.ld, sc.p[g], c.st));
            }
    }
    if (blk.shortcut) {
        Mat s2 = c.gemm_out(nq, blk.out_dim, sc.cols);
        Stat s2s = stat_buffer(c, nq, blk.out_dim);
        linear(c, sc, blk.shortcut, sc.cols, nullptr, s2, &s2s);
        norm_act(c, u2, 0.1f, y, &u2s, &s2, true, &s2s);
    } else {
        norm_act(c, u2, 0.1f, y, &u2s, &sc, false);
    }
    c.release(m);
    return y;
}

void edge_norm(Ctx& c, const float* cn, int ld_cn, int cw, const int* idx, int n, int k, float* emax, int ld_emax, float* out,
               int ld_out, void* sums, bool sums_ok, float* stats, void* ws, size_t wsb) {
    if (sums && sums_ok) {
        c.check(pcrcg_edgeconv_reduce_sums(cn, ld_cn, cn + cw, ld_cn, idx, n, k, cw, emax, ld_emax, sums, c.st));
        c.check(pcrcg_instnorm_apply_sums(emax, n, cw, ld_emax, sums, (double)n * (double)k, 1e-5f, nullptr, 0, nullptr, 0.2f, out,
                                          ld_out, c.st));
        return;
    }
    c.check(pcrcg_edgeconv_reduce(cn, ld_cn, cn + cw, ld_cn, idx, n, k, cw, 1e-5f, emax, ld_emax, stats, ws, wsb, c.st));
    c.check(pcrcg_instnorm_apply(emax, n, cw, ld_emax, stats, nullptr, 0, nullptr, 0.2f, out, ld_out, c.st));
}

void edge_norm_all(Ctx& c, const Mat& cn, int cw, int* const* idx, const int* n, const int* k, const Mat& e, const Mat& out,
                   void* const* sums, bool sums_ok, float* stats, void* ws, size_t wsb) {
    bool multi = sums_ok;
    EdgeCloud cl[GMAX];
    for (int g = 0; g < c.G; ++g) {
        multi = multi && sums[g] != nullptr;
        cl[g] = EdgeCloud{cn.p[g], cn.p[g] + cw, idx[g], e.p[g], static_cast<double*>(sums[g]), n[g], k[g]};
    }
    if (multi && edgeconv_rows_ok(cl, c.G, cn.ld, cn.ld, e.ld, cw)) {
        c.check(edgeconv_rows_multi(cl, c.G, cn.ld, cn.ld, e.ld, cw, true, nullptr, c.st));
        NormJob jobs[GMAX];
        bool al = c.G <= 4;
        for (int g = 0; g < c.G; ++g) {
            jobs[g] = NormJob{e.p[g], static_cast<const double*>(sums[g]), nullptr, nullptr, out.p[g], nullptr, nullptr, n[g],
                              (double)n[g] * (double)k[g]};
            al = al && ((reinterpret_cast<uintptr_t>(e.p[g]) | reinterpret_cast<uintptr_t>(out.p[g])) & 15) == 0 && n[g] > 0 && k[g] > 0;
        }
        if (al) {
            c.check(instnorm_apply_sums_multi(jobs, c.G, cw, e.ld, 1e-5f, 0, 0.2f, out.ld, false, c.st));
            return;
        }
        for (int g = 0; g < c.G; ++g)
            c.check(pcrcg_instnorm_apply_sums(e.p[g], n[g], cw, e.ld, sums[g], (double)n[g] * (double)k[g], 1e-5f, nullptr, 0, nullptr,
                                              0.2f, out.p[g], out.ld, c.st));
        return;
    }
    for (int g = 0; g < c.G; ++g)
        edge_norm(c, cn.p[g], cn.ld, cw, idx[g], n[g], k[g], e.p[g], e.ld, out.p[g], out.ld, sums[g], sums_ok, stats, ws, wsb);
}

Mat self_attention(Ctx& c, const pcrcg_model& mdl, const pcrcg_gnn_layer& gl, const float* const* coords, const Mat& f,
                   int* const* knn_given = nullptr) {
    const int ch = f.cols;
    Mat y = c.mat(f.rows, ch);
    const size_t m = c.mark();
    int kq[GMAX];
    int* idx[GMAX];
    for (int g = 0; g < c.G; ++g) {
        const int n = f.rows[g];
        kq[g] = mdl.knn_k < n - 1 ? mdl.knn_k : n - 1;
        idx[g] = knn_given ? knn_given[g] : static_cast<int*>(c.raw(sizeof(int) * (size_t)n * (kq[g] > 0 ? kq[g] : 1)));
    }
    Mat cat = c.mat(f.rows, 4 * ch);
    const size_t wsb = pcrcg_edgeconv_ws_bytes(2 * ch);
    void* ws = c.raw(wsb);
    float* stats = static_cast<float*>(c.raw(sizeof(float) * 4 * ch));
    Mat cn1 = c.gemm_out(f.rows, 2 * ch, ch), e1 = c.mat(f.rows, ch), cn2 = c.gemm_out(f.rows, 4 * ch, ch), e2 = c.mat(f.rows, 2 * ch);
    Mat x3 = c.gemm_out(f.rows, ch, 4 * ch);
    Stat x3s = stat_buffer(c, f.rows, ch);
    void *sums1[GMAX], *sums2[GMAX];
    for (int g = 0; g < c.G; ++g) {
        sums1[g] = gemm_colstats_sums_ok() ? c.zraw(2 * sizeof(double) * (size_t)ch) : nullptr;
        sums2[g] = gemm_colstats_sums_ok() ? c.zraw(2 * sizeof(double) * (size_t)(2 * ch)) : nullptr;
// ... 379 lines not shown
```

pcrcg_amd/csrc/train_runner.hip:

```cpp
#include <cmath>
#include <functional>
#include <mutex>
#include <vector>

#include "common.h"
#include "pcrcg_train.h"

namespace pcrcg {
int gemm_general(const float* a, int lda, int trans_a, const float* b, int ldb, int trans_b, float* c, int ldc, int m, int n,
                 int k, const float* row_scale, const float* bias, bool accumulate, hipStream_t st, int grad_operand = 0);
int gemm_bt_colstats(const float* a, int lda, const float* b, int ldb, float* c, int ldc, int m, int n, int k,
                     const float* row_scale, const float* bias, void* colstats, size_t colstats_bytes, int* h_chunks,
                     hipStream_t st, bool c_zeroed, bool colstats_sums);
int tr_scale_rows(const float* src, int ld_src, const float* s, float* dst, int rows, int cols, hipStream_t st);
int tr_add_lrelu(const float* a, int lda, const float* b, int ldb, float slope, float* y, int ldy, int rows, int cols,
                 hipStream_t st);
int tr_add_lrelu_bwd(const float* y, int ldy, const float* dy, int ld_dy, float slope, float* ga, int lga, float* gb, int lgb,
                     int rows, int cols, hipStream_t st);
int tr_add2d(const float* src, int ld_src, float* dst, int ld_dst, int rows, int cols, hipStream_t st);
int tr_bias_grad(const float* dy, int ld, int rows, int cols, float* db, hipStream_t st);
int tr_l2norm_bwd(const float* x, int ldx, const float* dy, int ld_dy, float* dx, int ld_dx, int rows, int cols, hipStream_t st);
int tr_sigmoid_bwd(const float* s, const float* ds, float* dx, int ld_dx, int rows, hipStream_t st);
int tr_dot_acc(const float* a, const float* b, long n, float scale, float* out, hipStream_t st);
bool instnorm_backward_sums_ok(const float* x, int n, int c, int ldx, const float* dy, int ld_dy, const float* dx, int ld_dx);
// ... 236 lines not shown
            one.stats_out = stats;
            t.check(instnorm_apply_sums_multi(&one, 1, x.cols, x.ld, 1e-5f, 0, slope, y.ld, false, t.st));
        } else {
            if (sums) t.check(pcrcg_instnorm_stats_from_partials(sums, 1, x.cols, (double)x.rows, 1e-5f, stats, t.st));
            else t.check(pcrcg_instnorm_stats(x.p, x.rows, x.cols, x.ld, 1e-5f, stats, ws, wsb, t.st));
            t.check(pcrcg_instnorm_apply(x.p, x.rows, x.cols, x.ld, stats, nullptr, 0, nullptr, slope, y.p, y.ld, t.st));
        }
    }
    double* bw_sums = x.rows <= 32 * 32 ? static_cast<double*>(t.grad.take(sizeof(double) * 2 * x.cols)) : nullptr;
    t.fits();
    t.need_scratch(bwb + 256);
    t.record([x, y, stats, slope, bwb, bw_sums](Tape& b) {
        if (!x.g) return;
        if (bw_sums && instnorm_backward_sums_ok(x.p, x.rows, x.cols, x.ld, y.g, y.ld, x.g, x.ld)) {
            b.check(instnorm_backward_sums(x.p, x.rows, x.cols, x.ld, stats, y.g, y.ld, slope, x.g, x.ld, bw_sums, b.st));
            return;
        }
        void* w = b.tmp((bwb + 3) / 4);
        b.check(pcrcg_instnorm_backward(x.p, x.rows, x.cols, x.ld, stats, y.g, y.ld, slope, x.g, x.ld, w, bwb, b.st));
    });
    return y;
}

TT add_lrelu(Tape& t, const TT& a, const TT& bb, float slope, TT* into = nullptr) {
    TT y = into ? *into : t.tensor(a.rows, a.cols);
    if (t.live()) t.check(tr_add_lrelu(a.p, a.ld, bb.p, bb.ld, slope, y.p, y.ld, a.rows, a.cols, t.st));
    t.record([a, bb, y, slope](Tape& b) {
        b.check(tr_add_lrelu_bwd(y.p, y.ld, y.g, y.ld, slope, a.g, a.ld, bb.g, bb.ld, a.rows, a.cols, b.st));
    });
    return y;
}

void copy_into(Tape& t, const TT& src, const TT& dst_slice) {
    if (t.live()) t.check(pcrcg_copy2d(src.p, src.ld, dst_slice.p, dst_slice.ld, src.rows, src.cols, t.st));
    t.record([src, dst_slice](Tape& b) {
        if (src.g && dst_slice.g) b.check(tr_add2d(dst_slice.g, dst_slice.ld, src.g, src.ld, src.rows, src.cols, b.st));
    });
}

TT kpconv(Tape& t, const pcrcg_batch& b, const pcrcg_block& blk, Wt w, const TT& x, const double** sums_out = nullptr) {
    if (sums_out) *sums_out = nullptr;
    const int l = blk.layer;
    const pcrcg_table& tab = blk.strided ? b.pools[l] : b.neighbors[l];
    const float* q = blk.strided ? b.points[l + 1] : b.points[l];
    const int nq = blk.strided ? b.n_points[l + 1] : b.n_points[l];
    const int ns = b.n_points[l], cin = x.cols, cout = blk.mid_dim, kc = PCRCG_KPOINTS * cin;
    TT y = t.tensor(nq, cout, true, 0, true);
    float* wf = static_cast<float*>(t.value_bytes(fbytes(nq, kc)));
    float* inv_n = static_cast<float*>(t.value_bytes(fbytes(nq, 1)));
    const size_t wsb = pcrcg_kpconv_ws_bytes(ns);
    void* ws = t.value_bytes(wsb);
    if (t.live()) {
        t.check(pcrcg_kpconv_aggregate(q, nq, b.points[l], ns, tab.idx, tab.cols, tab.ld, x.p, cin, blk.kp, blk.extent, wf,
                                       inv_n, ws, wsb, t.st));
        double* slot = (sums_out && blk.kp_wt && kc % 4 == 0) ? t.sums_slot(cout) : nullptr;
        if (slot) {
            int chunks = 0;
            t.check(gemm_bt_colstats(wf, kc, blk.kp_wt, kc, y.p, y.ld, nq, cout, kc, inv_n, nullptr, slot,
                                     (size_t)2 * cout * sizeof(double), &chunks, t.st, false, true));
            if (chunks == -1) *sums_out = slot;
        } else if (blk.kp_wt && kc % 4 == 0)
            t.check(gemm_general(wf, kc, 0, blk.kp_wt, kc, 1, y.p, y.ld, nq, cout, kc, inv_n, nullptr, false, t.st));
        else
            t.check(gemm_general(wf, kc, 0, w.p, cout, 0, y.p, y.ld, nq, cout, kc, inv_n, nullptr, false, t.st));
    }
    t.need_scratch(fbytes(nq, kc));
    float* dys = static_cast<float*>(t.value_bytes(fbytes(nq, cout)));
    const float* s_pts = b.points[l];
    const float* kp = blk.kp;
    const float extent = blk.extent;
    t.record([=](Tape& bk) {
        bk.check(tr_scale_rows(y.g, y.ld, inv_n, dys, nq, cout, bk.st));
        if (w.g)
            bk.check(gemm_general(wf, kc, 1, dys, cout, 0, w.g, cout, kc, cout, nq, nullptr, nullptr, true, bk.off_path(), 2));
        if (x.g) {
            float* d_wf = bk.tmp((size_t)(nq > 0 ? nq : 1) * kc + 64);
            bk.check(gemm_general(dys, cout, 0, w.p, cout, 1, d_wf, kc, nq, kc, cout, nullptr, nullptr, false, bk.st, 1));
            bk.check(pcrcg_kpconv_backward_dx(q, nq, s_pts, ns, tab.idx, tab.cols, tab.ld, d_wf, cin, kp, extent, x.g, bk.st));
        }
    });
    return y;
}

TT max_pool(Tape& t, const TT& x, const pcrcg_table& tab) {
    TT y = t.tensor(tab.rows, x.cols);
    if (t.live()) t.check(pcrcg_gather_max(x.p, x.rows, x.cols, tab.idx, tab.rows, tab.cols, tab.ld, y.p, t.st));
    t.record([x, y, tab](Tape& b) {
        if (x.g)
            b.check(pcrcg_gather_max_backward(x.p, x.rows, x.cols, tab.idx, tab.rows, tab.cols, tab.ld, y.p, y.g, x.g, b.st));
    });
    return y;
}

void closest_pool_into(Tape& t, const TT& x, const pcrcg_table& tab, const TT& dst) {
    if (t.live()) t.check(pcrcg_gather_first(x.p, x.rows, x.cols, tab.idx, tab.rows, tab.ld, dst.p, dst.ld, t.st));
    t.record([x, tab, dst](Tape& b) {
        if (x.g) b.check(pcrcg_gather_first_backward(dst.g, dst.ld, x.cols, tab.idx, tab.rows, tab.ld, x.rows, x.g, b.st));
    });
}

TT softmax_rows(Tape& t, const TT& s, float scale, float* scale_grad = nullptr) {
    float* raw = nullptr;
    if (scale_grad) raw = static_cast<float*>(t.value_bytes(fbytes(s.rows, s.cols)));
    if (t.live()) {
        if (raw) t.check(pcrcg_copy2d(s.p, s.ld, raw, s.cols, s.rows, s.cols, t.st));
        t.check(pcrcg_softmax_rows(s.p, s.rows, s.cols, s.ld, scale, t.st));
    }
    t.need_scratch(fbytes(s.rows, s.cols));
    t.record([s, scale, raw, scale_grad](Tape& b) {
        float* ds = b.tmp((size_t)(s.rows > 0 ? s.rows : 1) * s.cols + 64);
        b.check(pcrcg_softmax_rows_backward(s.p, s.ld, s.g, s.ld, s.rows, s.cols, scale, ds, s.cols, b.st));
        if (scale_grad)
            b.check(tr_dot_acc(ds, raw, (long)s.rows * s.cols, 1.0f / scale, scale_grad, b.st));
        b.check(pcrcg_copy2d(ds, s.cols, s.g, s.ld, s.rows, s.cols, b.st));
    });
    return s;
}

TT unary(Tape& t, const TT& x, Wt w, int ldw, int out, float slope) {
    const double* sums = nullptr;
    TT y = linear(t, x, w, ldw, Wt(), out, nullptr, &sums, true);
    return instnorm_lrelu(t, y, slope, nullptr, sums);
}

Wt wt(const float* p, const float* g) { Wt w; w.p = p; w.g = const_cast<float*>(g); return w; }

TT encoder_block(Tape& t, const pcrcg_batch& b, const pcrcg_block& blk, const pcrcg_block& gb, const TT& x) {
    const double* ksums = nullptr;
    if (blk.type == PCRCG_BLK_SIMPLE) {
        TT c0 = kpconv(t, b, blk, wt(blk.kp_w, gb.kp_w), x, &ksums);
        return instnorm_lrelu(t, c0, 0.1f, nullptr, ksums);
    }
    TT y = x;
    if (blk.unary1) y = unary(t, x, wt(blk.unary1, gb.unary1), x.cols, blk.mid_dim, 0.1f);
    {
        TT c1 = kpconv(t, b, blk, wt(blk.kp_w, gb.kp_w), y, &ksums);
        y = instnorm_lrelu(t, c1, 0.1f, nullptr, ksums);
    }
    y = unary(t, y, wt(blk.unary2, gb.unary2), blk.mid_dim, blk.out_dim, 1.0f);
    TT sc = blk.strided ? max_pool(t, x, b.pools[blk.layer]) : x;
    if (blk.shortcut) sc = unary(t, sc, wt(blk.shortcut, gb.shortcut), sc.cols, blk.out_dim, 1.0f);
    return add_lrelu(t, y, sc, 0.1f);
}

void edge_conv_core(Tape& t, const TT& ctr, const TT& nbr, int cout, const int* idx, int k, const TT& y) {
    const int n = ctr.rows;
    TT emax = t.tensor(n, cout, false);
    float* stats = static_cast<float*>(t.value_bytes(sizeof(float) * 2 * cout));
    const size_t wsb = pcrcg_edgeconv_ws_bytes(cout), bwb = pcrcg_edgeconv_backward_ws_bytes(cout);
    void* ws = t.value_bytes(wsb);
    if (t.live()) {
        t.check(pcrcg_edgeconv_reduce(ctr.p, ctr.ld, nbr.p, nbr.ld, idx, n, k, cout, 1e-5f, emax.p, emax.ld, stats, ws, wsb, t.st));
        t.check(pcrcg_instnorm_apply(emax.p, n, cout, emax.ld, stats, nullptr, 0, nullptr, 0.2f, y.p, y.ld, t.st));
    }
    t.need_scratch(bwb + fbytes(n, cout) + 512);
    t.record([=](Tape& b) {
        float* dy = b.tmp((size_t)n * cout + 64);
        b.check(pcrcg_copy2d(y.g, y.ld, dy, cout, n, cout, b.st));
        void* w = b.tmp((bwb + 3) / 4 + 64);
        b.check(pcrcg_edgeconv_backward(ctr.p, nbr.p, idx, n, k, cout, stats, dy, 0.2f, ctr.g, nbr.g, w, bwb, b.st));
    });
}
void edge_conv(Tape& t, const TT& f, Wt w_packed, int cout, int clouds, const int* rows_of, int* const* idx, const int* k,
               const TT& into) {
    const int cin = f.cols;
    Wt wc = w_packed, wn = w_packed;
    wn.p = w_packed.p + (long)cout * cin;
    wn.g = w_packed.g ? w_packed.g + (long)cout * cin : nullptr;
    TT ctr = linear(t, f, wc, cin, Wt(), cout), nbr = linear(t, f, wn, cin, Wt(), cout);
    for (int c = 0, r0 = 0; c < clouds; r0 += rows_of[c], ++c)
        edge_conv_core(t, rows(ctr, r0, rows_of[c]), rows(nbr, r0, rows_of[c]), cout, idx[c], k[c], rows(into, r0, rows_of[c]));
}

TT self_attention(Tape& t, const pcrcg_model& m, const pcrcg_gnn_layer& g, const pcrcg_gnn_layer& gg, int clouds,
                  const float* const* coords, const int* rows_of, const TT& f) {
    const int n = f.rows, ch = f.cols;
    int* idx[2];
    int k[2];
    for (int c = 0; c < clouds; ++c) {
        k[c] = m.knn_k < rows_of[c] - 1 ? m.knn_k : rows_of[c] - 1;
        idx[c] = static_cast<int*>(t.value_bytes(sizeof(int) * (size_t)rows_of[c] * (k[c] > 0 ? k[c] : 1) + 256));
        if (t.live()) t.check(pcrcg_knn(coords[c], rows_of[c], k[c], idx[c], t.st));
    }
    TT cat = t.tensor(n, 4 * ch);
    copy_into(t, f, cols(cat, 0, ch));
    TT s1 = cols(cat, ch, ch), s2 = cols(cat, 2 * ch, 2 * ch);
    edge_conv(t, f, wt(g.edge1, gg.edge1), ch, clouds, rows_of, idx, k, s1);
    edge_conv(t, s1, wt(g.edge2, gg.edge2), 2 * ch, clouds, rows_of, idx, k, s2);
    TT x3 = linear(t, cat, wt(g.conv3, gg.conv3), 4 * ch, Wt(), ch, nullptr, nullptr, true);
    TT out = t.tensor(n, ch);
    for (int c = 0, r0 = 0; c < clouds; r0 += rows_of[c], ++c) {
        TT oc = rows(out, r0, rows_of[c]);
        instnorm_lrelu(t, rows(x3, r0, rows_of[c]), 0.2f, &oc);
    }
    return out;
}

TT cross_attention(Tape& t, const pcrcg_model& m, const pcrcg_gnn_layer& g, const pcrcg_gnn_layer& gg, const TT& x,
                   const TT& src, TT* into = nullptr) {
    const int n = x.rows, ms = src.rows, ch = x.cols, h = m.heads, d = ch / h;
    TT q = linear(t, x, wt(g.wq, gg.wq), ch, wt(g.bq, gg.bq), ch);
    TT kk = linear(t, src, wt(g.wk, gg.wk), ch, wt(g.bk, gg.bk), ch);
    TT v = linear(t, src, wt(g.wv, gg.wv), ch, wt(g.bv, gg.bv), ch);
    TT msg = t.tensor(n, ch);
    const float scale = 1.0f / sqrtf((float)d);
    AttnCloud one{q.p, kk.p, v.p, msg.p, n, ms};
    const bool fused = !t.dry && q.g && kk.g && v.g && attention_mfma_ok(&one, 1, q.ld, kk.ld, v.ld, d) &&
                       attention_bwd_mfma_ok(n, ms, d, q.ld, kk.ld, v.ld, msg.ld);
    if (fused) {
        if (t.live()) t.check(attention_mfma_multi(&one, 1, q.ld, kk.ld, v.ld, msg.ld, h, d, scale, t.st));
        t.record([q, kk, v, msg, n, ms, h, d, scale](Tape& b) {
            b.check(attention_bwd_mfma(q.p, q.ld, kk.p, kk.ld, v.p, v.ld, msg.p, msg.ld, msg.g, msg.ld, q.g, q.ld, kk.g, kk.ld, v.g,
                                       v.ld, n, ms, h, d, scale, b.st));
        });
    } else {
        for (int i = 0; i < h; ++i) {
            TT qi = cols(q, i * d, d), ki = cols(kk, i * d, d), vi = cols(v, i * d, d), mi = cols(msg, i * d, d);
            TT prob = softmax_rows(t, matmul_bt(t, qi, ki), scale);
            matmul_nn(t, prob, vi, &mi);
        }
    }
    TT cat = t.tensor(n, 2 * ch);
    copy_into(t, x, cols(cat, 0, ch));
// ... 197 lines not shown
```

pcrcg_amd/ops.py:

```python
import ctypes

import torch

from . import _lib

_F32, _I32, _I64 = torch.float32, torch.int32, torch.int64


def _stream():
    return torch.cuda.current_stream().cuda_stream


def _dev(t, dtype, name):
    if not isinstance(t, torch.Tensor) or not t.is_cuda:
        raise RuntimeError(f"pcrcg_amd: `{name}` must be a tensor on a HIP device (no CPU fallback exists)")
    if t.dtype != dtype:
        raise RuntimeError(f"pcrcg_amd: `{name}` must have dtype {dtype}, got {t.dtype}")
    return t


def _rows(t, dtype, name):
    _dev(t, dtype, name)
    if t.dim() != 2:
        raise RuntimeError(f"pcrcg_amd: `{name}` must be 2-D")
# ... 404 lines not shown
    return f, (fmap, depth, valid)


def inject_frames(points, len_src, frames, channels=128, width=None):
    L = _lib.lib()
    pts = _dev(points, _F32, "points").contiguous()
    if pts.dim() != 2 or pts.shape[1] != 3:
        raise RuntimeError("pcrcg_amd.inject_frames: points must be [N, 3]")
    n = int(pts.shape[0])
    width = channels + 1 if width is None else int(width)
    if width < channels + 1:
        raise RuntimeError("pcrcg_amd.inject_frames: width must be at least channels + 1")
    if len(frames) > 6:
        raise RuntimeError("pcrcg_amd.inject_frames: at most 3 frames per cloud")
    arr = (ImageFrame * max(len(frames), 1))()
    keep = []
    for j, fr in enumerate(frames):
        arr[j], ts = frame_struct(fr, channels)
        keep.append(ts)
    x = torch.empty((n, width), dtype=_F32, device=pts.device)
    _lib.check(L.pcrcg_inject_frames(pts.data_ptr(), n, int(len_src), ctypes.cast(arr, ctypes.c_void_p), len(frames),
                                     channels, x.data_ptr(), width, _stream()), "pcrcg_inject_frames")
    return x


def kpconv_bf16(q_pts, s_pts, idx, x, kernel_points, weights, extent, intermediates=False):
    L = _lib.lib()
    q_pts, s_pts = _dev(q_pts, _F32, "q_pts").contiguous(), _dev(s_pts, _F32, "s_pts").contiguous()
    idx, ld_idx = _rows(idx, _I64, "idx")
    x = _dev(x, _F32, "x").contiguous()
    kernel_points = _dev(kernel_points, _F32, "kernel_points").contiguous()
    nq, ns, h, cin, cout = q_pts.shape[0], s_pts.shape[0], idx.shape[1], x.shape[1], weights.shape[2]
    if cin % 32:
        raise RuntimeError("pcrcg_amd.kpconv_bf16: cin must be a multiple of 32")
    kk = 15 * cin
    wt = _dev(weights, _F32, "weights").reshape(-1, cout).t().contiguous()
    xb = torch.empty((ns, cin), dtype=torch.int16, device=x.device)
    wfb = torch.empty((nq, kk), dtype=torch.int16, device=x.device)
    inv_n = torch.empty(nq, dtype=_F32, device=x.device)
    out = torch.empty((nq, cout), dtype=_F32, device=x.device)
    nbytes = L.pcrcg_kpconv_ws_bytes(ns)
    ws = _ws.get("kpconv", nbytes, x.device)
    _lib.check(L.pcrcg_kpconv_aggregate_bf16(q_pts.data_ptr(), nq, s_pts.data_ptr(), ns, idx.data_ptr(), h, ld_idx,
                                             x.data_ptr(), cin, kernel_points.data_ptr(), float(extent), xb.data_ptr(),
                                             wfb.data_ptr(), inv_n.data_ptr(), ws.data_ptr(), nbytes, _stream()),
               "pcrcg_kpconv_aggregate_bf16")
    _lib.check(L.pcrcg_gemm_bf16a_f32_colstats(wfb.data_ptr(), kk, wt.data_ptr(), kk, out.data_ptr(), cout, nq, cout, kk,
                                               inv_n.data_ptr(), None, None, 0, None, _stream()),
               "pcrcg_gemm_bf16a_f32_colstats")
    return (out, xb, wfb, inv_n) if intermediates else out


def gemm_bf16a(a_bf16, b, row_scale=None, bias=None):
    L = _lib.lib()
    if a_bf16.dtype != torch.bfloat16 or not a_bf16.is_cuda:
        raise RuntimeError("pcrcg_amd.gemm_bf16a: `a` must be a bfloat16 tensor on the HIP device")
    a = a_bf16.contiguous()
    b = _dev(b, _F32, "b").contiguous()
    m, k = a.shape
    n = b.shape[0]
    out = torch.empty((m, n), dtype=_F32, device=a.device)
    if row_scale is not None:
        row_scale = _dev(row_scale, _F32, "row_scale").contiguous()
    if bias is not None:
        bias = _dev(bias, _F32, "bias").contiguous()
    _lib.check(L.pcrcg_gemm_bf16a_f32_colstats(a.data_ptr(), k, b.data_ptr(), k, out.data_ptr(), n, m, n, k,
                                               _ptr(row_scale), _ptr(bias), None, 0, None, _stream()),
               "pcrcg_gemm_bf16a_f32_colstats")
    return out


def gather_max(x, idx):
    L = _lib.lib()
    x = _dev(x, _F32, "x").contiguous()
    idx, ld_idx = _rows(idx, _I64, "inds")
    ns, c = x.shape
    nq, h = idx.shape
    out = torch.empty((nq, c), dtype=_F32, device=x.device)
    _lib.check(L.pcrcg_gather_max(x.data_ptr(), ns, c, idx.data_ptr(), nq, h, ld_idx, out.data_ptr(), _stream()),
               "pcrcg_gather_max")
    return out


def gather_first(x, idx, out=None):
    L = _lib.lib()
    x = _dev(x, _F32, "x").contiguous()
    idx, ld_idx = _rows(idx, _I64, "inds")
    ns, c = x.shape
    nq = idx.shape[0]
    if out is None:
        out = torch.empty((nq, c), dtype=_F32, device=x.device)
    ld_out = out.stride(0) if nq > 1 else max(c, out.stride(0))
    if out.stride(1) != 1 and c > 1:
        raise RuntimeError("pcrcg_amd.gather_first: `out` must have unit inner stride")
    _lib.check(L.pcrcg_gather_first(x.data_ptr(), ns, c, idx.data_ptr(), nq, ld_idx, out.data_ptr(), ld_out,
                                    _stream()), "pcrcg_gather_first")
    return out


def instnorm_stats(x, eps=1e-5):
    L = _lib.lib()
    x, ldx = _rows(x, _F32, "x")
    n, c = x.shape
    stats = torch.empty(2 * c, dtype=_F32, device=x.device)
    nbytes = L.pcrcg_instnorm_ws_bytes(c)
    ws = _ws.get("instnorm", nbytes, x.device)
    _lib.check(L.pcrcg_instnorm_stats(x.data_ptr(), n, c, ldx, float(eps), stats.data_ptr(), ws.data_ptr(), nbytes,
                                      _stream()), "pcrcg_instnorm_stats")
    return stats


def instnorm_apply(x, stats, slope=1.0, res=None, res_stats=None, out=None):
    L = _lib.lib()
    x, ldx = _rows(x, _F32, "x")
    n, c = x.shape
    ldr = 0
    if res is not None:
        res, ldr = _rows(res, _F32, "res")
    if out is None:
        out = torch.empty((n, c), dtype=_F32, device=x.device)
    ldy = out.stride(0) if n > 1 else max(c, out.stride(0))
    _lib.check(L.pcrcg_instnorm_apply(x.data_ptr(), n, c, ldx, stats.data_ptr(), _ptr(res), ldr, _ptr(res_stats),
                                      float(slope), out.data_ptr(), ldy, _stream()), "pcrcg_instnorm_apply")
    return out


def instnorm_colsums(x):
    L = _lib.lib()
    x, ldx = _rows(x, _F32, "x")
    sums = torch.zeros((2, x.shape[1]), dtype=torch.float64, device=x.device)
    if x.shape[0] > 0:
        _lib.check(L.pcrcg_instnorm_colsums(x.data_ptr(), x.shape[0], x.shape[1], ldx, sums.data_ptr(), _stream()),
                   "pcrcg_instnorm_colsums")
    return sums


def instnorm_apply_sums(x, sums, slope=1.0, res=None, res_sums=None, eps=1e-5, out=None, count=None):
    L = _lib.lib()
    x, ldx = _rows(x, _F32, "x")
    n, c = x.shape
    if sums.dtype != torch.float64 or tuple(sums.shape) != (2, c) or not sums.is_contiguous():
        raise RuntimeError("pcrcg_amd.instnorm_apply_sums: sums must be a contiguous float64 [2, c] tensor")
    ldr = 0
    if res is not None:
        res, ldr = _rows(res, _F32, "res")
    if out is None:
        out = torch.empty((n, c), dtype=_F32, device=x.device)
    ldy = out.stride(0) if n > 1 else max(c, out.stride(0))
    _lib.check(L.pcrcg_instnorm_apply_sums(x.data_ptr(), n, c, ldx, sums.data_ptr(), float(n if count is None else count),
                                           float(eps), _ptr(res), ldr,
                                           _ptr(res_sums), float(slope), out.data_ptr(), ldy, _stream()),
               "pcrcg_instnorm_apply_sums")
    return out


def instnorm_lrelu(x, slope, eps=1e-5):
    return instnorm_apply(x, instnorm_stats(x, eps), slope)


def knn(coords, k):
    L = _lib.lib()
    coords = _dev(coords, _F32, "coords").contiguous()
    n = coords.shape[0]
    idx = torch.empty((n, k), dtype=_I32, device=coords.device)
    _lib.check(L.pcrcg_knn(coords.data_ptr(), n, int(k), idx.data_ptr(), _stream()), "pcrcg_knn")
    return idx
# ... 89 lines not shown
```

pcrcg_amd/pyramid.py:

```python
import os

import numpy as np
import torch

from . import ops
from .config import as_config

_I32 = torch.int32


def _layer_plan(config):
    arch = config.architecture
    r_normal = config.first_subsampling_dl * config.conv_radius
    levels, layer_blocks = [], []
    for i, block in enumerate(arch):
        if "global" in block or "upsample" in block:
            break
        if not ("pool" in block or "strided" in block):
            layer_blocks.append(block)
            if i < len(arch) - 1 and "upsample" not in arch[i + 1]:
                continue
        deform_conv = any("deformable" in b for b in layer_blocks[:-1])
        r_conv = r_normal * config.deform_radius / config.conv_radius if deform_conv else r_normal
        pooled = "pool" in block or "strided" in block
# ... 178 lines not shown

    def set_side_streams(self, sub=None, forest=None):
        self.side = (sub, forest)
        self.cfg.side_stream = sub.cuda_stream if sub is not None else None
        self.cfg.side_stream2 = forest.cuda_stream if forest is not None else None

    def restore(self, deferred, slot):
        self._lib.check(self._lib.lib().pcrcg_pyramid_restore_run(self._ct.byref(deferred), self.status.data_ptr() + 4 * slot,
                                                                  torch.cuda.current_stream().cuda_stream),
                        "pcrcg_pyramid_restore_run")

    def build(self, points, lengths, fresh_arena=False, defer_restore=False, group=0):
        ct, L = self._ct, self._lib.lib()
        parts = isinstance(points, (list, tuple))
        pts_l = [p.to(torch.float32).contiguous() for p in (points if parts else [points])]
        lens_l = [l.to(_I32).contiguous() for l in (lengths if parts else [lengths])]
        if not all(p.is_cuda for p in pts_l):
            raise RuntimeError("pcrcg_amd.build_pyramid: points must be on a HIP device (no CPU path)")
        pts, lens = pts_l[0], lens_l[0]
        n0, nb = sum(int(p.shape[0]) for p in pts_l), sum(int(l.shape[0]) for l in lens_l)
        stream = torch.cuda.current_stream().cuda_stream
        if group and nb % group:
            raise RuntimeError("pcrcg_amd.NativePyramid: the number of clouds is not a multiple of `group`")
        self.cfg.group = int(group)
        nbatch = nb // group if group else 1
        h_len = (ct.c_int * (self.levels * nb))()
        from .runner import PyramidRestore
        deferred = PyramidRestore() if defer_restore else None
        slot = self.calls % self.STATUS_RING
        self.calls += 1
        while True:
            self.cfg.shrink = float(self.shrink)
            need = L.pcrcg_pyramid_ws_bytes(n0, nb, ct.byref(self.cfg))
            if need == 0:
                raise RuntimeError("pcrcg_pyramid_ws_bytes rejected the configuration")
            arena = self.arena
            if fresh_arena or arena is None or arena.numel() < need or arena.device != pts.device:
                arena = torch.empty(int(need), dtype=torch.uint8, device=pts.device)
                if not fresh_arena:
                    self.arena = arena
            b = (self._Batch * nbatch)() if group else self._Batch()
            if parts:
                k = len(pts_l)
                pp = (ct.c_void_p * k)(*[p.data_ptr() for p in pts_l])
                lp = (ct.c_void_p * k)(*[l.data_ptr() for l in lens_l])
                pn = (ct.c_int * k)(*[int(p.shape[0]) for p in pts_l])
                ln = (ct.c_int * k)(*[int(l.shape[0]) for l in lens_l])
                rc = L.pcrcg_pyramid_build_parts(pp, pn, lp, ln, k, ct.byref(self.cfg), arena.data_ptr(), arena.numel(),
                                                 self.scratch.data_ptr(), ct.byref(b), h_len,
                                                 self.status.data_ptr() + 4 * slot,
                                                 ct.byref(deferred) if defer_restore else None, stream)
            else:
                rc = L.pcrcg_pyramid_build(pts.data_ptr(), n0, lens.data_ptr(), nb, ct.byref(self.cfg), arena.data_ptr(),
                                           arena.numel(), self.scratch.data_ptr(), ct.byref(b), h_len,
                                           self.status.data_ptr() + 4 * slot,
                                           ct.byref(deferred) if defer_restore else None, stream)
            if rc == -2 and self.shrink < 1.0:
                self.shrink = 1.0
                continue
            self._lib.check(rc, "pcrcg_pyramid_build")
            break
        lens_h = [[int(h_len[l * nb + i]) for i in range(nb)] for l in range(self.levels)]
        if defer_restore:
            return b, arena, lens_h, slot, deferred
        return b, arena, lens_h, slot

    def as_dict(self, b, arena, lens_h, part=None):
        base = arena.data_ptr()
        if part is not None:
            lens_h = [row[part[0]:part[0] + part[1]] for row in lens_h]
        nb = len(lens_h[0])

        def view(ptr, nbytes, dtype):
            off = ptr - base
            return arena[off:off + nbytes].view(dtype)

        def table(t):
            if t.idx and t.rows > 0 and t.cols > 0:
                return view(t.idx, t.rows * t.ld * 8, torch.int64).view(t.rows, t.ld)[:, :t.cols]
            if t.idx and t.rows > 0:
                return torch.zeros((t.rows, 0), dtype=torch.int64, device=arena.device)
            return torch.zeros((0, 1), dtype=torch.int64, device=arena.device)

        out = {"points": [], "neighbors": [], "pools": [], "upsamples": [], "stack_lengths": []}
        for l in range(b.n_levels):
            n = b.n_points[l]
            out["points"].append(view(b.points[l], n * 12, torch.float32).view(n, 3))
            out["neighbors"].append(table(b.neighbors[l]))
            out["pools"].append(table(b.pools[l]))
            out["upsamples"].append(table(b.upsamples[l]))
            out["stack_lengths"].append(view(b.stack_lengths[l], nb * 4, _I32))
        out["features"] = view(b.features, b.n_points[0] * 4, torch.float32).view(-1, 1)
        out["stack_lengths_host"] = lens_h
        return out


def build_pyramid_native(points, lengths, config, neighborhood_limits, tie_order=None, side_streams=None):
    nat = NativePyramid(config, neighborhood_limits, tie_order)
    if side_streams is not None:
        nat.set_side_streams(*side_streams)
    b, arena, lens_h, slot = nat.build(points, lengths, fresh_arena=True)
    torch.cuda.current_stream().synchronize()
    check_tie_status(int(nat.status[slot]))
    out = nat.as_dict(b, arena, lens_h)
    out["tie_status"] = None
    return out


def _point2node(nodes, points):
    d = -2.0 * points @ nodes.t()
    d = d + (points ** 2).sum(-1, keepdim=True) + (nodes ** 2).sum(-1)[None, :]
    return torch.clamp(d, min=1e-12).argmin(1)


def _node_visibility(nodes, points, visible_idx):
    p2n = _point2node(nodes, points)
    tot = torch.ones(nodes.shape[0], device=nodes.device)
    idx, cts = torch.unique(p2n, return_counts=True)
    tot[idx] = cts.float()
    vis_mask = torch.zeros(points.shape[0], device=nodes.device)
    vis_mask[visible_idx] = 1.0
    vis_pts = vis_mask.nonzero().squeeze(1)
    vis = torch.zeros(nodes.shape[0], device=nodes.device)
    idx_, cts_ = torch.unique(p2n[vis_pts], return_counts=True)
    vis[idx_] = cts_.float()
    return vis / tot, p2n


def collate_fn_descriptor(list_data, config, neighborhood_limits, device=None, side_streams=None):
    assert len(list_data) == 1
    device = torch.device(device if device is not None else "cuda")
    item = list_data[0]
    src = torch.as_tensor(np.asarray(item["src_pcd"]), dtype=torch.float32).to(device)
    tgt = torch.as_tensor(np.asarray(item["tgt_pcd"]), dtype=torch.float32).to(device)
    points = torch.cat([src, tgt], 0)
    lengths = torch.tensor([src.shape[0], tgt.shape[0]], dtype=_I32, device=device)
    out = build_pyramid(points, lengths, config, neighborhood_limits, side_streams=side_streams)
    feats = np.concatenate([np.asarray(item["src_feats"]), np.asarray(item["tgt_feats"])], 0)
    out["features"] = torch.as_tensor(feats, dtype=torch.float32).to(device)
    out["rot"] = torch.as_tensor(np.asarray(item["rot"])).to(device)
    out["trans"] = torch.as_tensor(np.asarray(item["trans"])).to(device)
    corr = item["correspondences"]
    out["correspondences"] = corr
    out["src_pcd_raw"], out["tgt_pcd_raw"] = src, tgt
    out["sample"] = item.get("sample")
    nodes = out["points"][-1]
    n_src = out["stack_lengths_host"][-1][0]
    corr_t = (corr if isinstance(corr, torch.Tensor) else torch.as_tensor(np.asarray(corr))).to(device).long()
    src_vis, src_p2n = _node_visibility(nodes[:n_src], src, corr_t[:, 0])
    tgt_vis, tgt_p2n = _node_visibility(nodes[n_src:], tgt, corr_t[:, 1])
    out["node_overlap_gt"] = torch.cat([src_vis, tgt_vis])
    out["points2node"] = torch.cat([src_p2n, tgt_p2n])
    for key in item.keys():
        if key not in out and key not in ("src_pcd", "tgt_pcd", "src_feats", "tgt_feats"):
            out[key] = item[key]
    return out


def calibrate_neighbors(pairs, config, keep_ratio=0.8, samples_threshold=2000):
    config = as_config(config)
    hist_n = int(np.ceil(4 / 3 * np.pi * (config.deform_radius + 1) ** 3))
    hists = np.zeros((config.num_layers, hist_n), dtype=np.int64)
    for points, lengths in pairs:
        b = build_pyramid(points, lengths, config, [hist_n] * config.num_layers, want_counts=True)
        for l, cnt in enumerate(b["neighbor_counts"]):
            c = torch.clamp(cnt.long(), max=hist_n)
            hists[l] += torch.bincount(c, minlength=hist_n + 1)[:hist_n].cpu().numpy()
        if hists.sum(1).min() > samples_threshold:
# ... 4 lines not shown
```

pcrcg_amd/runner.py:

```python
import ctypes
import threading

import torch

from . import _lib
from .blocks import (LastUnaryBlock, NearestUpsampleBlock, ResnetBottleneckBlock, SimpleBlock, UnaryBlock,
                     aligned_weight)
from .gcn import AttentionalPropagation, SelfAttention

MAX_LEVELS, MAX_BLOCKS, MAX_GNN = 8, 32, 8
BLK_SIMPLE, BLK_RESNETB, BLK_UNARY, BLK_LAST_UNARY, BLK_UPSAMPLE = range(5)
_fp = ctypes.c_void_p


class Block(ctypes.Structure):
    _fields_ = [("type", ctypes.c_int), ("layer", ctypes.c_int), ("strided", ctypes.c_int),
                ("in_dim", ctypes.c_int), ("out_dim", ctypes.c_int), ("mid_dim", ctypes.c_int),
                ("extent", ctypes.c_float), ("kp", _fp), ("kp_w", _fp), ("kp_wt", _fp), ("kp_w_pad", _fp),
                ("cin_pad", ctypes.c_int), ("unary1", _fp), ("unary2", _fp),
                ("shortcut", _fp), ("mlp", _fp), ("mlp_ld", ctypes.c_int),
                ("mlp_skip", _fp), ("mlp_skip_ld", ctypes.c_int), ("skip_dim", ctypes.c_int)]


class GnnLayer(ctypes.Structure):
    _fields_ = [("cross", ctypes.c_int), ("edge1", _fp), ("edge2", _fp), ("conv3", _fp),
                ("wq", _fp), ("bq", _fp), ("wk", _fp), ("bk", _fp), ("wv", _fp), ("bv", _fp),
                ("wm", _fp), ("bm", _fp), ("w0", _fp), ("b0", _fp), ("w3", _fp), ("b3", _fp)]


class Model(ctypes.Structure):
    _fields_ = [("n_enc", ctypes.c_int), ("n_dec", ctypes.c_int), ("n_gnn", ctypes.c_int),
                ("enc", Block * MAX_BLOCKS), ("dec", Block * MAX_BLOCKS), ("gnn", GnnLayer * MAX_GNN),
                ("enc_skip", ctypes.c_int * MAX_BLOCKS), ("dec_concat", ctypes.c_int * MAX_BLOCKS),
                ("enc_out_dim", ctypes.c_int), ("gnn_dim", ctypes.c_int), ("heads", ctypes.c_int),
                ("knn_k", ctypes.c_int), ("final_dim", ctypes.c_int),
                ("bottle_w", _fp), ("bottle_b", _fp), ("proj_gnn_w", _fp), ("proj_gnn_b", _fp),
                ("proj_score_w", _fp), ("proj_score_b", _fp), ("temperature", ctypes.c_float),
                ("feature_bf16", ctypes.c_int)]


class Table(ctypes.Structure):
    _fields_ = [("idx", _fp), ("rows", ctypes.c_int), ("cols", ctypes.c_int), ("ld", ctypes.c_int)]


class Batch(ctypes.Structure):
    _fields_ = [("n_levels", ctypes.c_int), ("points", _fp * MAX_LEVELS), ("n_points", ctypes.c_int * MAX_LEVELS),
                ("neighbors", Table * MAX_LEVELS), ("pools", Table * MAX_LEVELS), ("upsamples", Table * MAX_LEVELS),
                ("features", _fp), ("feat_dim", ctypes.c_int), ("len_src_c", ctypes.c_int),
                ("stack_lengths", _fp * MAX_LEVELS)]


class PyramidCfg(ctypes.Structure):
    _fields_ = [("n_levels", ctypes.c_int), ("r_conv", ctypes.c_float * MAX_LEVELS), ("r_pool", ctypes.c_float * MAX_LEVELS),
                ("dl", ctypes.c_float * MAX_LEVELS), ("has_conv", ctypes.c_int * MAX_LEVELS),
                ("pooled", ctypes.c_int * MAX_LEVELS), ("limit", ctypes.c_int * MAX_LEVELS), ("tie_order", ctypes.c_int),
                ("group", ctypes.c_int), ("up_nearest", ctypes.c_int), ("shrink", ctypes.c_double), ("side_stream", _fp),
                ("side_stream2", _fp)]


from .ops import ReorderJob as ReorderJobC


class PyramidRestore(ctypes.Structure):
    _fields_ = [("njobs", ctypes.c_int), ("jobs", ReorderJobC * 12), ("tie_status", _fp)]


class Outputs(ctypes.Structure):
    _fields_ = [("feats_f", _fp), ("scores_overlap", _fp), ("scores_saliency", _fp)]


_bound = False


def _bind():
    global _bound
    L = _lib.lib()
    if not _bound:
        _bound = True
    return L


def _dense(t):
    t = t.detach()
    if t.dtype != torch.float32 or not t.is_cuda:
        raise RuntimeError("pcrcg_amd.runner: parameters must be float32 tensors on a HIP device")
    return t.contiguous()


class Runner:

    def __init__(self, model):
        self.model = model
        self.sig = None
        self.desc = None
        self.keep = []
        self.ws = {}
        self._lock = threading.Lock()
        self._params = None
        self._built = None
        self._seen = set()
        self._retired = []

    def __deepcopy__(self, memo):
        return None

    def __reduce__(self):
        return (type(None), ())

    def _signature(self):
        if self._params is None:
            self._params = list(self.model.parameters())
        return (bool(getattr(self.model, "feature_bf16", False)),) + tuple(
            (p.data_ptr(), p._version) for p in self._params)

    def invalidate(self):
        with self._lock:
            self._params, self.sig = None, None

    def _w(self, t):
        t = _dense(t)
        self.keep.append(t)
        return t.data_ptr()

    def _kp_weights(self, blk, kp):
        cin = kp.in_channels
        blk.kp_w = self._w(kp.weights.data)
        w = kp.weights.data
        if cin % 4 == 0 or cin < 4:
            blk.kp_w_pad, blk.cin_pad = None, 0
        else:
            cp = (cin + 3) // 4 * 4
            w = torch.zeros((kp.weights.shape[0], cp, kp.out_channels), dtype=torch.float32, device=kp.weights.device)
# ... 77 lines not shown
                return self.desc
            old_keep, self.keep = self.keep, []
            try:
                d = self._build()
            except BaseException:
                self.keep = old_keep
                raise
            self._built = torch.cuda.Event()
            self._built.record()
            self._seen = set()
            if old_keep:
                evs = [torch.cuda.ExternalStream(st, device=torch.device("cuda", di)).record_event() for (di, st) in self.ws]
                self._retired.append((old_keep, evs))
            self._retired = [(k, evs) for (k, evs) in self._retired if not all(e.query() for e in evs)]
            self.desc, self.sig = d, sig
            return d

    def _build(self):
        m = self.model
        d = Model()
        d.n_enc, d.n_dec, d.n_gnn = len(m.encoder_blocks), len(m.decoder_blocks), len(m.gnn.layers)
        if d.n_enc > MAX_BLOCKS or d.n_dec > MAX_BLOCKS or d.n_gnn > MAX_GNN:
            raise RuntimeError("pcrcg_amd.runner: architecture too deep for the descriptor")
        for i, mod in enumerate(m.encoder_blocks):
            self._fill_block(d.enc[i], mod)
            d.enc_skip[i] = int(i in m.encoder_skips)
        cur_dim = m.bottle.out_channels + 2
        for j, mod in enumerate(m.decoder_blocks):
            self._fill_block(d.dec[j], mod)
            d.dec_concat[j] = int(j in m.decoder_concats)
            if isinstance(mod, (UnaryBlock, LastUnaryBlock)):
                if j in m.decoder_concats and mod.in_dim > cur_dim:
                    cs = mod.in_dim - cur_dim
                    ws = mod.mlp.weight.data[:, cur_dim:]
                    pad = (-cs) % 4
                    ws = torch.nn.functional.pad(ws, (0, pad)).contiguous() if pad else ws.contiguous()
                    self.keep.append(ws)
                    d.dec[j].mlp_skip, d.dec[j].mlp_skip_ld, d.dec[j].skip_dim = ws.data_ptr(), cs + pad, cs
                cur_dim = mod.out_dim
        heads = None
        for i, layer in enumerate(m.gnn.layers):
            self._fill_gnn(d.gnn[i], layer, heads)
            if isinstance(layer, AttentionalPropagation):
                heads = layer.attn.num_heads
            else:
                d.knn_k = layer.k
        d.heads = heads or 1
        d.enc_out_dim, d.gnn_dim, d.final_dim = m.bottle.in_channels, m.bottle.out_channels, m.final_feats_dim
        d.bottle_w, d.bottle_b = self._w(m.bottle.weight.data.squeeze(-1)), self._w(m.bottle.bias.data)
        d.proj_gnn_w, d.proj_gnn_b = self._w(m.proj_gnn.weight.data.squeeze(-1)), self._w(m.proj_gnn.bias.data)
        d.proj_score_w, d.proj_score_b = (self._w(m.proj_score.weight.data.squeeze(-1)),
                                          self._w(m.proj_score.bias.data))
        d.temperature = float(torch.exp(m.epsilon.detach()).item()) + 0.03
        d.feature_bf16 = int(bool(getattr(m, "feature_bf16", False)))
        return d

    @staticmethod
    def _table(dst, t, keep):
        if t.numel() == 0:
            dst.idx, dst.rows, dst.cols, dst.ld = None, int(t.shape[0]), 0, 1
            return
        if t.dtype != torch.int64 or not t.is_cuda:
            raise RuntimeError("pcrcg_amd.runner: index tables must be int64 tensors on the device")
        if t.shape[1] > 1 and t.stride(1) != 1:
            t = t.contiguous()
        keep.append(t)
        dst.idx, dst.rows, dst.cols = t.data_ptr(), int(t.shape[0]), int(t.shape[1])
        dst.ld = int(t.stride(0)) if t.shape[0] > 1 else int(t.shape[1])

    def batch_struct(self, batch):
        keep = []
        b = Batch()
        pts = batch["points"]
        b.n_levels = len(pts)
        for l, p in enumerate(pts):
            p = p.contiguous()
            if p.dtype != torch.float32 or not p.is_cuda:
                raise RuntimeError("pcrcg_amd.runner: points must be float32 tensors on the device")
            keep.append(p)
            b.points[l], b.n_points[l] = p.data_ptr(), int(p.shape[0])
            self._table(b.neighbors[l], batch["neighbors"][l], keep)
            self._table(b.pools[l], batch["pools"][l], keep)
            self._table(b.upsamples[l], batch["upsamples"][l], keep)
        feats = batch["features"].to(torch.float32).contiguous()
        keep.append(feats)
        b.features, b.feat_dim = feats.data_ptr(), int(feats.shape[1])
        if "stack_lengths_host" in batch:
            b.len_src_c = int(batch["stack_lengths_host"][-1][0])
        else:
            b.len_src_c = int(batch["stack_lengths"][-1][0])
        return b, keep, feats.device

    def forward(self, batch):
        b, keep, dev = self.batch_struct(batch)
        return self.launch(b, dev)

    def launch_group(self, batches, n, dev, start=0):
        L = _bind()
        desc = self.descriptor()
        outs, o = [], (Outputs * n)()
        first = ctypes.byref(batches[start])
        for g in range(n):
            n0 = batches[start + g].n_points[0]
            out = {"feats_f": torch.empty((n0, desc.final_dim), dtype=torch.float32, device=dev),
                   "scores_overlap": torch.empty(n0, dtype=torch.float32, device=dev),
                   "scores_saliency": torch.empty(n0, dtype=torch.float32, device=dev)}
            o[g].feats_f, o[g].scores_overlap, o[g].scores_saliency = (out["feats_f"].data_ptr(), out["scores_overlap"].data_ptr(),
                                                                      out["scores_saliency"].data_ptr())
            outs.append(out)
        nbytes = L.pcrcg_kpfcnn_group_ws_bytes(ctypes.byref(desc), first, n)
        if nbytes == 0:
            raise RuntimeError("pcrcg_kpfcnn_group_ws_bytes rejected the descriptors: " + (L.pcrcg_last_error() or b"").decode())
        cur = torch.cuda.current_stream()
        stream = cur.cuda_stream
        key = (dev.index if dev.index is not None else torch.cuda.current_device(), stream)
        with self._lock:
            ws = self.ws.get(key)
            if ws is None or ws.numel() < nbytes:
                ws = torch.empty(int(nbytes * 1.25), dtype=torch.uint8, device=dev)
                self.ws[key] = ws
            if key not in self._seen and self._built is not None:
                cur.wait_event(self._built)
                self._seen.add(key)
        _lib.check(L.pcrcg_kpfcnn_forward_group(ctypes.byref(desc), first, o, n, ws.data_ptr(), ws.numel(), stream),
                   "pcrcg_kpfcnn_forward_group")
        return outs

    def launch(self, b, dev):
        L = _bind()
        desc = self.descriptor()
        n0 = b.n_points[0]
        out = {"feats_f": torch.empty((n0, desc.final_dim), dtype=torch.float32, device=dev),
               "scores_overlap": torch.empty(n0, dtype=torch.float32, device=dev),
               "scores_saliency": torch.empty(n0, dtype=torch.float32, device=dev)}
        o = Outputs(out["feats_f"].data_ptr(), out["scores_overlap"].data_ptr(), out["scores_saliency"].data_ptr())
        nbytes = L.pcrcg_kpfcnn_ws_bytes(ctypes.byref(desc), ctypes.byref(b))
        if nbytes == 0:
            raise RuntimeError("pcrcg_kpfcnn_ws_bytes rejected the descriptors: "
                               + (L.pcrcg_last_error() or b"").decode())
        cur = torch.cuda.current_stream()
        stream = cur.cuda_stream
        key = (dev.index if dev.index is not None else torch.cuda.current_device(), stream)
        with self._lock:
            ws = self.ws.get(key)
            if ws is None or ws.numel() < nbytes:
                ws = torch.empty(int(nbytes * 1.25), dtype=torch.uint8, device=dev)
                self.ws[key] = ws
            if key not in self._seen and self._built is not None:
                cur.wait_event(self._built)
                self._seen.add(key)
        _lib.check(L.pcrcg_kpfcnn_forward(ctypes.byref(desc), ctypes.byref(b), ctypes.byref(o), ws.data_ptr(),
                                          ws.numel(), stream), "pcrcg_kpfcnn_forward")
        return out
```

Before: 607.5.

## Order max-pool queries by grid cell and stage shared neighbor rows in LDS

Adds a pass during pyramid construction that records pooled query rows grouped by their grid cell, and a new gather-max kernel that handles 16 spatially close queries per block. The kernel deduplicates their neighbor indices with a shared-memory hash, stages each unique source row once in LDS, and computes the max from LDS. It is meant to cut redundant global reads of overlapping neighborhoods in strided pooling. The cost is an extra ordering kernel plus a memset, hash and atomic overhead, and a fallback path when a piece has more than 192 unique rows.

Result: slower. 582.6 (-4.1%).

```diff
diff --git a/include/pcrcg.h b/include/pcrcg.h
--- a/include/pcrcg.h
+++ b/include/pcrcg.h
@@ -107,6 +107,8 @@
 
 int pcrcg_gather_max(const float* x, int ns, int c, const int64_t* idx, int nq, int h, int ld_idx,
                      float* out, void* stream);
+struct pcrcg_gather_max_job;
+int pcrcg_gather_max_ordered(const struct pcrcg_gather_max_job* h_jobs, int n_jobs, int c, void* stream);
 int pcrcg_gather_first(const float* x, int ns, int c, const int64_t* idx, int nq, int ld_idx, float* out,
                        int ld_out, void* stream);
 size_t pcrcg_instnorm_ws_bytes(int c);
@@ -225,6 +227,13 @@
 
 typedef struct pcrcg_table { const int64_t* idx; int rows, cols, ld; } pcrcg_table;
 
+typedef struct pcrcg_pool_order { const int* order; const int* groups; int max_groups; } pcrcg_pool_order;
+typedef struct pcrcg_gather_max_job {
+    const float* x; const int64_t* idx; float* out;
+    int ns, nq, h, ld_idx;
+    pcrcg_pool_order order;
+} pcrcg_gather_max_job;
+
 typedef struct pcrcg_batch {
     int n_levels;
     const float* points[PCRCG_MAX_LEVELS];
@@ -234,6 +243,7 @@
     int feat_dim;
     int len_src_c;
     const int* stack_lengths[PCRCG_MAX_LEVELS];
+    pcrcg_pool_order pool_order[PCRCG_MAX_LEVELS];
 } pcrcg_batch;
 
 typedef struct pcrcg_outputs {
diff --git a/pcrcg_amd/_lib.py b/pcrcg_amd/_lib.py
--- a/pcrcg_amd/_lib.py
+++ b/pcrcg_amd/_lib.py
@@ -66,6 +66,7 @@
     "pcrcg_instnorm_stats_from_partials": (c_int, [c_void_p, c_int, c_int, ctypes.c_double, c_float, c_void_p,
                                                    c_void_p]),
     "pcrcg_gather_max": (c_int, [c_void_p, c_int, c_int, c_void_p, c_int, c_int, c_int, c_void_p, c_void_p]),
+    "pcrcg_gather_max_ordered": (c_int, [c_void_p, c_int, c_int, c_void_p]),
     "pcrcg_gather_first": (c_int, [c_void_p, c_int, c_int, c_void_p, c_int, c_int, c_void_p, c_int, c_void_p]),
     "pcrcg_instnorm_ws_bytes": (c_size_t, [c_int]),
     "pcrcg_instnorm_stats": (c_int, [c_void_p, c_int, c_int, c_int, c_float, c_void_p, c_void_p, c_size_t, c_void_p]),
diff --git a/pcrcg_amd/csrc/common.h b/pcrcg_amd/csrc/common.h
--- a/pcrcg_amd/csrc/common.h
+++ b/pcrcg_amd/csrc/common.h
@@ -111,6 +111,11 @@
 
 struct GatherJob { const float* x; const int64_t* idx; float* out; int ns, nq, h, ld_idx; };
 int gather_max_multi(const GatherJob* jobs, int count, int c, hipStream_t st);
+struct GatherOrder { const int* order; const int* groups; int max_groups; };
+bool gather_max_ordered_ok(const GatherJob* jobs, const GatherOrder* ord, int count, int c);
+int gather_max_ordered_multi(const GatherJob* jobs, const GatherOrder* ord, int count, int c, hipStream_t st);
+size_t pool_order_group_words(int nq_cap, int nb, int group);
+int pool_order_pass(const void* qgrid, int nq_cap, int nb, int group, int* order, void* groups, hipStream_t st);
 int heads_multi(const float* const* x, const int* rows, int count, int ld, int fd, float* const* feats, float* const* s_ov,
                 float* const* s_sal, hipStream_t st);
 int copy2d_multi(const float* const* src, float* const* dst, const int* rows, int count, int ld_src, int ld_dst, int cols,
diff --git a/pcrcg_amd/csrc/pointops.hip b/pcrcg_amd/csrc/pointops.hip
--- a/pcrcg_amd/csrc/pointops.hip
+++ b/pcrcg_amd/csrc/pointops.hip
@@ -45,6 +45,128 @@
             any = true;
         }
         out[(long)q * c + cc] = m;
+    }
+}
+
+constexpr int kOrdQ = 16;
+constexpr int kOrdH = 64;
+constexpr int kOrdRows = 192;
+constexpr int kOrdCols = 16;
+constexpr int kOrdHash = 2048;
+struct GatherOrdMulti {
+    const float* x[4]; const long long* idx[4]; float* out[4]; const int* order[4]; const int* groups[4];
+    int ns[4], nq[4], h[4], ld_idx[4], max_groups[4];
+};
+__global__ void __launch_bounds__(256) k_gather_max_ordered(GatherOrdMulti mm, int c4) {
+    __shared__ float4 s_stage[kOrdRows * kOrdCols];
+    __shared__ unsigned short s_slot[kOrdQ * kOrdH];
+    __shared__ int s_row[kOrdRows];
+    __shared__ int s_q[kOrdQ];
+    __shared__ int s_rows;
+    static_assert(sizeof(int) * kOrdHash <= sizeof(float4) * kOrdRows * kOrdCols, "the id table shares the staging buffer");
+    static_assert(kOrdQ * kOrdH <= 4 * 256 && kOrdHash >= 2 * kOrdQ * kOrdH && kOrdRows < 0xFFFF, "piece geometry");
+    int* s_tab = reinterpret_cast<int*>(s_stage);
+    const int g = blockIdx.y;
+    const float* __restrict__ x = mm.x[g];
+    const long long* __restrict__ idx = mm.idx[g];
+    float* __restrict__ out = mm.out[g];
+    const int* __restrict__ order = mm.order[g];
+    const int* __restrict__ groups = mm.groups[g];
+    const int ns = mm.ns[g], nq = mm.nq[g], h = mm.h[g], ld_idx = mm.ld_idx[g];
+    const int c = 4 * c4;
+    const int t = threadIdx.x, qi = t >> 4, cl = t & 15;
+    int ngroups = mm.max_groups[g] > 0 ? groups[1] : 0;
+    if (ngroups > mm.max_groups[g]) ngroups = mm.max_groups[g];
+    for (int grp = blockIdx.x; grp < ngroups; grp += gridDim.x) {
+        int g_start = groups[2 + 2 * grp], g_count = groups[3 + 2 * grp];
+        if (g_start < 0 || g_count <= 0 || g_start >= nq) continue;
+        if (g_count > nq - g_start) g_count = nq - g_start;
+        for (int p0 = g_start; p0 < g_start + g_count; p0 += kOrdQ) {
+            const int nqp = min(kOrdQ, g_start + g_count - p0);
+            __syncthreads();
+            if (t < nqp) {
+                const int q = order[p0 + t];
+                s_q[t] = q >= 0 && q < nq ? q : -1;
+            }
+            if (t == 0) s_rows = 0;
+            for (int i = t; i < kOrdHash; i += 256) s_tab[i] = -1;
+            __syncthreads();
+            int place[4];
+#pragma unroll
+            for (int u = 0; u < 4; ++u) {
+                const int e = t + 256 * u;
+                place[u] = -1;
+                if (e < nqp * h) {
+                    const int eq = e / h, q = s_q[eq];
+                    const long long i = q >= 0 ? idx[(long)q * ld_idx + (e - eq * h)] : -1;
+                    if (i >= 0 && i < ns) {
+                        const int id = (int)i;
+                        unsigned s = ((unsigned)id * 2654435761u) >> 21;
+                        for (;;) {
+                            const int prev = atomicCAS(&s_tab[s], -1, id);
+                            if (prev == -1 || prev == id) break;
+                            s = (s + 1) & (kOrdHash - 1);
+                        }
+                        place[u] = (int)s;
+                    }
+                }
+            }
+            __syncthreads();
+            for (int i = t; i < kOrdHash; i += 256) {
+                const int id = s_tab[i];
+                if (id >= 0) {
+                    const int r = atomicAdd(&s_rows, 1);
+                    if (r < kOrdRows) s_row[r] = id;
+                    s_tab[i] = r;
+                }
+            }
+            __syncthreads();
+#pragma unroll
+            for (int u = 0; u < 4; ++u) {
+                const int e = t + 256 * u;
+                if (e < nqp * h) s_slot[e] = place[u] >= 0 ? (unsigned short)s_tab[place[u]] : (unsigned short)0xFFFF;
+            }
+            __syncthreads();
+            const int nrows = s_rows;
+            const int q = qi < nqp ? s_q[qi] : -1;
+            if (nrows <= kOrdRows) {
+                for (int cb = 0; cb < c4; cb += kOrdCols) {
+                    const int col = cb + cl;
+                    if (cb > 0) __syncthreads();
+                    for (int r = qi; r < nrows; r += 16)
+                        s_stage[r * kOrdCols + cl] = col < c4 ? reinterpret_cast<const float4*>(x + (long)s_row[r] * c)[col]
+                                                              : make_float4(0.f, 0.f, 0.f, 0.f);
+                    __syncthreads();
+                    if (q >= 0 && col < c4) {
+                        float4 m = make_float4(0.f, 0.f, 0.f, 0.f);
+                        bool any = false;
+                        const unsigned short* sl = s_slot + qi * h;
+                        for (int j = 0; j < h; ++j) {
+                            const unsigned r = sl[j];
+                            float4 v = make_float4(0.f, 0.f, 0.f, 0.f);
+                            if (r != 0xFFFFu) v = s_stage[r * kOrdCols + cl];
+                            if (!any) { m = v; any = true; }
+                            else { m.x = fmaxf(m.x, v.x); m.y = fmaxf(m.y, v.y); m.z = fmaxf(m.z, v.z); m.w = fmaxf(m.w, v.w); }
+                        }
+                        reinterpret_cast<float4*>(out + (long)q * c)[col] = m;
+                    }
+                }
+            } else if (q >= 0) {
+                const long long* row = idx + (long)q * ld_idx;
+                for (int col = cl; col < c4; col += 16) {
+                    float4 m = make_float4(0.f, 0.f, 0.f, 0.f);
+                    bool any = false;
+                    for (int j = 0; j < h; ++j) {
+                        const long long i = row[j];
+                        float4 v = make_float4(0.f, 0.f, 0.f, 0.f);
+                        if (i >= 0 && i < ns) v = reinterpret_cast<const float4*>(x + i * c)[col];
+                        if (!any) { m = v; any = true; }
+                        else { m.x = fmaxf(m.x, v.x); m.y = fmaxf(m.y, v.y); m.z = fmaxf(m.z, v.z); m.w = fmaxf(m.w, v.w); }
+                    }
+                    reinterpret_cast<float4*>(out + (long)q * c)[col] = m;
+                }
+            }
+        }
     }
 }
 
@@ -398,6 +520,37 @@
     return PCRCG_OK;
 }
 
+bool gather_max_ordered_ok(const GatherJob* jobs, const GatherOrder* ord, int count, int c) {
+    if (!jobs || !ord || count < 1 || count > 4 || c < 4 || c % 4 != 0) return false;
+    for (int g = 0; g < count; ++g) {
+        const GatherJob& j = jobs[g];
+        if (!ord[g].order || !ord[g].groups || ord[g].max_groups < 0 || j.h < 1 || j.h > kOrdH || j.ld_idx < j.h) return false;
+        if (j.nq > 0 && ((reinterpret_cast<uintptr_t>(j.x) | reinterpret_cast<uintptr_t>(j.out)) & 15) != 0) return false;
+    }
+    return true;
+}
+int gather_max_ordered_multi(const GatherJob* jobs, const GatherOrder* ord, int count, int c, hipStream_t st) {
+    PCRCG_CHECK_ARG(gather_max_ordered_ok(jobs, ord, count, c));
+    GatherOrdMulti mm;
+    int nq_max = 0;
+    for (int g = 0; g < 4; ++g) {
+        const int k = g < count ? g : 0;
+        const GatherJob& j = jobs[k];
+        PCRCG_CHECK_ARG(j.ns >= 0 && j.nq >= 0 && (j.nq == 0 || (j.x && j.idx && j.out)));
+        mm.x[g] = j.x; mm.idx[g] = reinterpret_cast<const long long*>(j.idx); mm.out[g] = j.out;
+        mm.order[g] = ord[k].order; mm.groups[g] = ord[k].groups;
+        mm.ns[g] = j.ns; mm.nq[g] = g < count ? j.nq : 0; mm.h[g] = j.h; mm.ld_idx[g] = j.ld_idx;
+        mm.max_groups[g] = g < count && j.nq > 0 ? ord[k].max_groups : 0;
+        if (g < count && j.nq > nq_max) nq_max = j.nq;
+    }
+    if (nq_max == 0) return PCRCG_OK;
+    int blocks = (nq_max + 5) / 6;
+    if (blocks > 1024) blocks = 1024;
+    hipLaunchKernelGGL(k_gather_max_ordered, dim3(blocks, count), dim3(256), 0, st, mm, c / 4);
+    PCRCG_CHECK_LAUNCH();
+    return PCRCG_OK;
+}
+
 int instnorm_colsums_multi(const float* const* x, double* const* sums, const int* n, int count, int c, int ldx, hipStream_t st) {
     PCRCG_CHECK_ARG(count >= 1 && count <= 4 && c >= 1 && ldx >= c);
     ColsMulti mm;
@@ -429,6 +582,20 @@
     PCRCG_CHECK_ARG(x && idx && out);
     const GatherJob one{x, idx, out, ns, nq, h, ld_idx};
     return gather_max_multi(&one, 1, c, as_stream(stream));
+}
+
+int pcrcg_gather_max_ordered(const pcrcg_gather_max_job* h_jobs, int n_jobs, int c, void* stream) {
+    PCRCG_CHECK_ARG(h_jobs && n_jobs >= 1 && n_jobs <= 4 && c >= 1);
+    GatherJob jobs[4];
+    GatherOrder ord[4];
+    for (int g = 0; g < n_jobs; ++g) {
+        const pcrcg_gather_max_job& j = h_jobs[g];
+        PCRCG_CHECK_ARG(j.ns >= 0 && j.nq >= 0 && j.h >= 1 && j.ld_idx >= j.h && (j.nq == 0 || (j.x && j.idx && j.out)));
+        jobs[g] = GatherJob{j.x, j.idx, j.out, j.ns, j.nq, j.h, j.ld_idx};
+        ord[g] = GatherOrder{j.order.order, j.order.groups, j.order.max_groups};
+    }
+    if (gather_max_ordered_ok(jobs, ord, n_jobs, c)) return gather_max_ordered_multi(jobs, ord, n_jobs, c, as_stream(stream));
+    return gather_max_multi(jobs, n_jobs, c, as_stream(stream));
 }
 
 int pcrcg_gather_first(const float* x, int ns, int c, const int64_t* idx, int nq, int ld_idx, float* out,
diff --git a/pcrcg_amd/csrc/pyramid.hip b/pcrcg_amd/csrc/pyramid.hip
--- a/pcrcg_amd/csrc/pyramid.hip
+++ b/pcrcg_amd/csrc/pyramid.hip
@@ -234,6 +234,8 @@
 
     void* carried = nullptr;
     float carried_r = 0.f;
+    int* pool_rows[PCRCG_MAX_LEVELS] = {};
+    unsigned long long* pool_groups[PCRCG_MAX_LEVELS] = {};
     PCRCG_PROPAGATE(order(st, sub_st));
     if (!one_forest) PCRCG_PROPAGATE(build_forest(0));
     else if (L == 1) PCRCG_PROPAGATE(build_forest(0));
@@ -272,6 +274,10 @@
             void* up_grid = nullptr;
             PCRCG_PROPAGATE(build_grid(sub, m, sub_len, 2 * r_pool, &up_grid));
             PCRCG_PROPAGATE(add_table(1, l, l + 1, grid, up_grid, r_pool, sub, sub_len, m, n, lens, limit, l));
+            pool_rows[l] = A.take<int>((size_t)m);
+            pool_groups[l] = static_cast<unsigned long long*>(A.raw(sizeof(unsigned long long) * pool_order_group_words(m, nb, group)));
+            if (!A.ok()) return PCRCG_EWORKSPACE;
+            if (!dry) PCRCG_PROPAGATE(pool_order_pass(up_grid, m, nb, group, pool_rows[l], pool_groups[l], st));
             PCRCG_PROPAGATE(add_table(2, l, l, up_grid, grid, 2 * r_pool, pts, lens, n, m, sub_len, cfg->up_nearest ? 1 : limit, l + 1));
             carried = up_grid;
             carried_r = 2 * r_pool;
@@ -338,7 +344,14 @@
             o.neighbors[l] = pcrcg_table{nullptr, rows, 0, 1};
             o.pools[l] = pcrcg_table{nullptr, 0, 0, 1};
             o.upsamples[l] = pcrcg_table{nullptr, 0, 0, 1};
-        }
+            o.pool_order[l] = pcrcg_pool_order{nullptr, nullptr, 0};
+            if (pool_rows[l] && l + 1 < L) {
+                int q0, qn;
+                group_rows(l + 1, p, &q0, &qn);
+                o.pool_order[l] = pcrcg_pool_order{pool_rows[l] + q0, reinterpret_cast<const int*>(pool_groups[l] + q0 + p), qn};
+            }
+        }
+        for (int l = L; l < PCRCG_MAX_LEVELS; ++l) o.pool_order[l] = pcrcg_pool_order{nullptr, nullptr, 0};
     }
     pcrcg_pyramid_restore local;
     pcrcg_pyramid_restore& R = deferred ? *deferred : local;
diff --git a/pcrcg_amd/csrc/radius.hip b/pcrcg_amd/csrc/radius.hip
--- a/pcrcg_amd/csrc/radius.hip
+++ b/pcrcg_amd/csrc/radius.hip
@@ -896,6 +896,39 @@
     return radius_query_pass(q, nq, qlen, ns, slen, nb, group, radius, sgrid, cols, out_idx, out_count, out_max_count, status,
                              out_tie_rows, out_tie_count, st, 2);
 }
+
+namespace {
+constexpr int kPoolGroupRows = 16;
+__global__ void __launch_bounds__(256) k_pool_order(GridView g, int group, int* __restrict__ order, u64* __restrict__ groups) {
+    const int j = blockIdx.x * blockDim.x + threadIdx.x;
+    if (j >= (int)(g.hdr->cursor >> 32)) return;
+    const int4 ci = g.cinfo[j];
+    const int p = group > 0 ? ci.z / group : 0;
+    const int row0 = group > 0 ? g.soff[p * group] : 0;
+    const int pieces = (ci.x + kPoolGroupRows - 1) / kPoolGroupRows;
+    u64* head = groups + row0 + p;
+    const u64 got = atomicAdd(head, ((u64)(unsigned)pieces << 32) | (u64)(unsigned)ci.x);
+    const int at = (int)(unsigned)got, gi = (int)(got >> 32);
+    for (int k = 0; k < ci.x; ++k) order[row0 + at + k] = __float_as_int(g.spts[ci.y + k].w) - row0;
+    for (int k = 0; k < pieces; ++k) {
+        const int left = ci.x - k * kPoolGroupRows;
+        head[1 + gi + k] = (u64)(unsigned)(at + k * kPoolGroupRows) | ((u64)(unsigned)(left < kPoolGroupRows ? left : kPoolGroupRows) << 32);
+    }
+}
+}
+
+size_t pool_order_group_words(int nq_cap, int nb, int group) { return (size_t)(nq_cap > 0 ? nq_cap : 0) + (group > 0 ? nb / group : 1); }
+
+int pool_order_pass(const void* qgrid, int nq_cap, int nb, int group, int* order, void* groups, hipStream_t st) {
+    PCRCG_CHECK_ARG(qgrid && order && groups && nq_cap >= 0 && nb >= 1 && group >= 0);
+    PCRCG_CHECK_HIP(hipMemsetAsync(groups, 0, sizeof(u64) * pool_order_group_words(nq_cap, nb, group), st));
+    if (nq_cap == 0) return PCRCG_OK;
+    bool ok;
+    GridView gq = grid_view(const_cast<void*>(qgrid), grid_bytes(nq_cap, nb), nq_cap, nb, &ok);
+    hipLaunchKernelGGL(k_pool_order, dim3((nq_cap + 255) / 256), dim3(256), 0, st, gq, group, order, static_cast<u64*>(groups));
+    PCRCG_CHECK_LAUNCH();
+    return PCRCG_OK;
+}
 }
 
 extern "C" {
diff --git a/pcrcg_amd/csrc/runner.hip b/pcrcg_amd/csrc/runner.hip
--- a/pcrcg_amd/csrc/runner.hip
+++ b/pcrcg_amd/csrc/runner.hip
@@ -493,11 +493,15 @@
         sc = c.mat(nq, feats.cols);
         if (c.live() && c.G <= 4) {
             GatherJob jobs[GMAX];
+            GatherOrder ord[GMAX];
             for (int g = 0; g < c.G; ++g) {
                 const pcrcg_table& t = B.b[g]->pools[blk.layer];
+                const pcrcg_pool_order& o = B.b[g]->pool_order[blk.layer];
                 jobs[g] = GatherJob{feats.p[g], t.idx, sc.p[g], feats.rows[g], nq[g], t.cols, t.ld};
-            }
-            c.check(gather_max_multi(jobs, c.G, feats.cols, c.st));
+                ord[g] = GatherOrder{o.order, o.groups, o.max_groups};
+            }
+            if (gather_max_ordered_ok(jobs, ord, c.G, feats.cols)) c.check(gather_max_ordered_multi(jobs, ord, c.G, feats.cols, c.st));
+            else c.check(gather_max_multi(jobs, c.G, feats.cols, c.st));
         } else if (c.live())
             for (int g = 0; g < c.G; ++g) {
                 const pcrcg_table& t = B.b[g]->pools[blk.layer];
diff --git a/pcrcg_amd/csrc/train_runner.hip b/pcrcg_amd/csrc/train_runner.hip
--- a/pcrcg_amd/csrc/train_runner.hip
+++ b/pcrcg_amd/csrc/train_runner.hip
@@ -342,9 +342,14 @@
     return y;
 }
 
-TT max_pool(Tape& t, const TT& x, const pcrcg_table& tab) {
+TT max_pool(Tape& t, const TT& x, const pcrcg_table& tab, const pcrcg_pool_order& po) {
     TT y = t.tensor(tab.rows, x.cols);
-    if (t.live()) t.check(pcrcg_gather_max(x.p, x.rows, x.cols, tab.idx, tab.rows, tab.cols, tab.ld, y.p, t.st));
+    if (t.live() && tab.rows > 0) {
+        const GatherJob job{x.p, tab.idx, y.p, x.rows, tab.rows, tab.cols, tab.ld};
+        const GatherOrder ord{po.order, po.groups, po.max_groups};
+        if (tab.cols >= 1 && gather_max_ordered_ok(&job, &ord, 1, x.cols)) t.check(gather_max_ordered_multi(&job, &ord, 1, x.cols, t.st));
+        else t.check(pcrcg_gather_max(x.p, x.rows, x.cols, tab.idx, tab.rows, tab.cols, tab.ld, y.p, t.st));
+    }
     t.record([x, y, tab](Tape& b) {
         if (x.g)
             b.check(pcrcg_gather_max_backward(x.p, x.rows, x.cols, tab.idx, tab.rows, tab.cols, tab.ld, y.p, y.g, x.g, b.st));
@@ -398,7 +403,7 @@
         y = instnorm_lrelu(t, c1, 0.1f, nullptr, ksums);
     }
     y = unary(t, y, wt(blk.unary2, gb.unary2), blk.mid_dim, blk.out_dim, 1.0f);
-    TT sc = blk.strided ? max_pool(t, x, b.pools[blk.layer]) : x;
+    TT sc = blk.strided ? max_pool(t, x, b.pools[blk.layer], b.pool_order[blk.layer]) : x;
     if (blk.shortcut) sc = unary(t, sc, wt(blk.shortcut, gb.shortcut), sc.cols, blk.out_dim, 1.0f);
     return add_lrelu(t, y, sc, 0.1f);
 }
diff --git a/pcrcg_amd/ops.py b/pcrcg_amd/ops.py
--- a/pcrcg_amd/ops.py
+++ b/pcrcg_amd/ops.py
@@ -510,6 +510,49 @@
     return out
 
 
+class PoolOrderC(ctypes.Structure):
+    _fields_ = [("order", ctypes.c_void_p), ("groups", ctypes.c_void_p), ("max_groups", ctypes.c_int)]
+
+
+class GatherMaxJobC(ctypes.Structure):
+    _fields_ = [("x", ctypes.c_void_p), ("idx", ctypes.c_void_p), ("out", ctypes.c_void_p), ("ns", ctypes.c_int),
+                ("nq", ctypes.c_int), ("h", ctypes.c_int), ("ld_idx", ctypes.c_int), ("order", PoolOrderC)]
+
+
+def pool_order_groups(cuts, device):
+    cuts = [int(v) for v in cuts]
+    words = [0, len(cuts) - 1]
+    for a, b in zip(cuts[:-1], cuts[1:]):
+        words += [a, b - a]
+    return torch.tensor(words, dtype=_I32, device=device)
+
+
+def gather_max_ordered(jobs):
+    L = _lib.lib()
+    arr = (GatherMaxJobC * len(jobs))()
+    outs, keep = [], []
+    c = int(jobs[0][0].shape[1])
+    for k, (x, idx, order, groups) in enumerate(jobs):
+        x = _dev(x, _F32, "x").contiguous()
+        idx, ld_idx = _rows(idx, _I64, "inds")
+        if int(x.shape[1]) != c:
+            raise RuntimeError("pcrcg_amd.gather_max_ordered: the jobs of one launch share one feature width")
+        out = torch.empty((idx.shape[0], c), dtype=_F32, device=x.device)
+        j = arr[k]
+        j.x, j.idx, j.out = x.data_ptr(), idx.data_ptr(), out.data_ptr()
+        j.ns, j.nq, j.h, j.ld_idx = int(x.shape[0]), int(idx.shape[0]), int(idx.shape[1]), ld_idx
+        if order is not None and groups is not None:
+            order, groups = _dev(order, _I32, "order").contiguous(), _dev(groups, _I32, "groups").contiguous()
+            if order.numel() < idx.shape[0] or groups.numel() < 2:
+                raise RuntimeError("pcrcg_amd.gather_max_ordered: order needs one entry per table row, groups a header")
+            j.order.order, j.order.groups = order.data_ptr(), groups.data_ptr()
+            j.order.max_groups = groups.numel() // 2 - 1
+        keep += [x, idx, order, groups]
+        outs.append(out)
+    _lib.check(L.pcrcg_gather_max_ordered(arr, len(jobs), c, _stream()), "pcrcg_gather_max_ordered")
+    return outs
+
+
 def gather_first(x, idx, out=None):
     L = _lib.lib()
     x = _dev(x, _F32, "x").contiguous()
diff --git a/pcrcg_amd/pyramid.py b/pcrcg_amd/pyramid.py
--- a/pcrcg_amd/pyramid.py
+++ b/pcrcg_amd/pyramid.py
@@ -284,8 +284,14 @@
                 return torch.zeros((t.rows, 0), dtype=torch.int64, device=arena.device)
             return torch.zeros((0, 1), dtype=torch.int64, device=arena.device)
 
-        out = {"points": [], "neighbors": [], "pools": [], "upsamples": [], "stack_lengths": []}
+        def pool_order(o):
+            if not o.order or not o.groups:
+                return None
+            return (view(o.order, o.max_groups * 4, _I32), view(o.groups, 8 * (1 + o.max_groups), _I32))
+
+        out = {"points": [], "neighbors": [], "pools": [], "upsamples": [], "stack_lengths": [], "pool_orders": []}
         for l in range(b.n_levels):
+            out["pool_orders"].append(pool_order(b.pool_order[l]))
             n = b.n_points[l]
             out["points"].append(view(b.points[l], n * 12, torch.float32).view(n, 3))
             out["neighbors"].append(table(b.neighbors[l]))
diff --git a/pcrcg_amd/runner.py b/pcrcg_amd/runner.py
--- a/pcrcg_amd/runner.py
+++ b/pcrcg_amd/runner.py
@@ -43,11 +43,15 @@
     _fields_ = [("idx", _fp), ("rows", ctypes.c_int), ("cols", ctypes.c_int), ("ld", ctypes.c_int)]
 
 
+class PoolOrder(ctypes.Structure):
+    _fields_ = [("order", _fp), ("groups", _fp), ("max_groups", ctypes.c_int)]
+
+
 class Batch(ctypes.Structure):
     _fields_ = [("n_levels", ctypes.c_int), ("points", _fp * MAX_LEVELS), ("n_points", ctypes.c_int * MAX_LEVELS),
                 ("neighbors", Table * MAX_LEVELS), ("pools", Table * MAX_LEVELS), ("upsamples", Table * MAX_LEVELS),
                 ("features", _fp), ("feat_dim", ctypes.c_int), ("len_src_c", ctypes.c_int),
-                ("stack_lengths", _fp * MAX_LEVELS)]
+                ("stack_lengths", _fp * MAX_LEVELS), ("pool_order", PoolOrder * MAX_LEVELS)]
 
 
 class PyramidCfg(ctypes.Structure):
@@ -291,6 +295,16 @@
             self._table(b.neighbors[l], batch["neighbors"][l], keep)
             self._table(b.pools[l], batch["pools"][l], keep)
             self._table(b.upsamples[l], batch["upsamples"][l], keep)
+            po = batch["pool_orders"][l] if "pool_orders" in batch else None
+            if po is not None and b.pools[l].idx:
+                order, groups = po
+                if order.dtype != torch.int32 or groups.dtype != torch.int32 or not order.is_cuda or not groups.is_cuda \
+                        or order.numel() < b.pools[l].rows or groups.numel() < 2:
+                    raise RuntimeError("pcrcg_amd.runner: pool_orders entries are (order [rows], groups) int32 device tensors")
+                order, groups = order.contiguous(), groups.contiguous()
+                keep += [order, groups]
+                b.pool_order[l].order, b.pool_order[l].groups = order.data_ptr(), groups.data_ptr()
+                b.pool_order[l].max_groups = groups.numel() // 2 - 1
         feats = batch["features"].to(torch.float32).contiguous()
         keep.append(feats)
         b.features, b.feat_dim = feats.data_ptr(), int(feats.shape[1])
```
